# Sirui-Xu/InterDiff

Measured on AMD Instinct MI355X. Metric: denoising frame-steps/sec (denoising-steps/sec x B x T frames), higher is better.
Workload: dtype f32 (every contraction of the denoiser -- feed-forward block, QKV projection, self-attention, row-block contractions and the two token GEMMs: every fp32 operand as two f16 planes, 3 f16 MFMAs per product, fp32 accumulate; SMPL and everything else fp32 MFMA / VALU)

## Files before the change

include/interdiff_hip.h:

```cpp
#ifndef INTERDIFF_HIP_H
#define INTERDIFF_HIP_H

#include <stddef.h>
#include <stdint.h>

#ifdef __cplusplus
extern "C" {
#endif

#define IDF_OK            0
#define IDF_E_INVAL      -22
#define IDF_E_NOMEM      -12
#define IDF_E_LAUNCH     -5

int         interdiff_abi_version(void);
const char *interdiff_build_info(void);

int interdiff_rotation_6d_to_matrix   (const float *d6, float *m,  int64_t n, void *stream);
int interdiff_matrix_to_rotation_6d   (const float *m,  float *d6, int64_t n, void *stream);
int interdiff_matrix_to_axis_angle    (const float *m,  float *aa, int64_t n, void *stream);
int interdiff_axis_angle_to_matrix    (const float *aa, float *m,  int64_t n, void *stream);
int interdiff_axis_angle_to_quaternion(const float *aa, float *q,  int64_t n, void *stream);
int interdiff_rotation_6d_to_axis_angle(const float *d6, float *aa, int64_t n, void *stream);

typedef struct {
    int32_t V, J, n_betas, KB, S;
    const float   *blend;
    const float   *jt;
    const float   *js;
    const int32_t *parents;
    const int32_t *skin_idx;
    const float   *skin_w;
} idf_smpl_model;

size_t interdiff_smpl_workspace_bytes(const idf_smpl_model *m, int64_t N);
int interdiff_smpl_forward(const idf_smpl_model *m, const float *pose, const float *betas,
                           const float *trans, int64_t N, float *verts, float *jtr,
                           float *v_posed, void *ws, size_t ws_bytes, void *stream);

int interdiff_vertex_normals(const float *verts, int64_t N, int32_t V, const int32_t *faces,
                             const int32_t *adj_ptr, const int32_t *adj_face,
                             const int32_t *adj_corner, float *normals, void *stream);
int interdiff_nn_argmin(const float *q, int32_t Pq, const float *r, int32_t Pr, int64_t N,
                        int32_t *idx, void *stream);
int interdiff_point2point_signed(const float *x, int32_t P1, const float *y, int32_t P2, int64_t N,
                                 const float *x_normals, const float *y_normals,
                                 float *y2x_signed, float *x2y_signed, int32_t *yidx, int32_t *xidx,
                                 float *y2x, float *x2y, void *stream);

#define IDF_MDM_LAYERS 8
#define IDF_MDM_D      256
#define IDF_MDM_FF     1024
#define IDF_MDM_HEADS  4
#define IDF_MDM_NQ     10
#define IDF_MDM_MEM    10
#define IDF_MDM_MEM_MAX 16
#define IDF_FFN_SLICES 5

typedef struct {
    int64_t is_qan;
    int64_t sa_in_w, sa_in_b, sa_out_w, sa_out_b;
    int64_t qc, wk;
    int64_t ca_q_w, ca_q_b;
    int64_t ca_kv_w, ca_kv_b;
    int64_t ca_out_w, ca_out_b;
    int64_t ff1_w, ff1_b, ff2_w, ff2_b;
    int64_t ffn_pack;
    int64_t ffn_b1p;
    int64_t sa_in_pack;
    int64_t sa_out_frag;
    int64_t ln_w[3], ln_b[3];
    int64_t ffn_pack_h2;
    int64_t sa_in_pack_h2;
    int64_t qc_h2;
    int64_t rb_h2_ok;
    int64_t sa_out_frag_h2;
    int64_t qkv_bounds_ok;
} idf_mdm_layer;

typedef struct {
    int32_t C;
    int32_t n_steps;
    const float *arena;
    int64_t in_w, in_b;
    int64_t out_w, out_b;
    int64_t temb_table;
    int64_t pe;
    int32_t max_T, has_encoder;
    idf_mdm_layer layer[IDF_MDM_LAYERS];
    idf_mdm_layer enc_layer[IDF_MDM_LAYERS];
    int32_t tune[8];
    int64_t out_w_h2, in_w_h2;
    int64_t tail_h2_ok;
    int32_t mem_len;
    int32_t rb_tokens;
} idf_mdm_weights;

int interdiff_gemm_f32(const float *A, int32_t lda, const float *W, const float *bias, const float *resid, float *C,
                       int32_t ldc, int32_t M, int32_t N, int32_t K, int32_t epi, int32_t cfg, void *stream);

int interdiff_mdm_ffn(const idf_mdm_weights *w, int32_t layer, int32_t encoder, const float *x2, int32_t M, float *parts, void *stream);
size_t interdiff_mdm_memctx_floats_for(int32_t B, int32_t mem_len);

size_t interdiff_mdm_memctx_floats(int32_t B);
size_t interdiff_mdm_workspace_bytes(int32_t B, int32_t T);
int interdiff_mdm_prepare_memory(const idf_mdm_weights *w, const float *cond, int32_t B,
                                 float *memctx, void *ws, size_t ws_bytes, void *stream);
int interdiff_mdm_forward(const idf_mdm_weights *w, const float *memctx, const float *x,
                          const int64_t *ts, int32_t B, int32_t T, float *x0,
                          void *ws, size_t ws_bytes, void *stream);

typedef struct {
    int64_t w[3], b[3];
    int32_t c[4];
} idf_pn_mlp;

typedef struct {
    const float *arena;
    idf_pn_mlp sa1[2];
    idf_pn_mlp sa2[2];
    int64_t lin_w, lin_b;
} idf_pointnet2;

int interdiff_pointnet2_encode(const idf_pointnet2 *pn, const float *obj_points, int32_t B, int32_t P, float *out,
                               void *stream);
size_t interdiff_mdm_encode_workspace_bytes(int32_t B, int32_t Tp);
int interdiff_mdm_encode(const idf_mdm_weights *w, const float *pc, const float *x_past, int32_t B, int32_t Tp,
                         float *cond, void *ws, size_t ws_bytes, void *stream);

int interdiff_inpaint(float *x0, const float *gt, const uint8_t *mask, int64_t n, void *stream);
int interdiff_posterior_step(float *x, const float *x0, const float *noise, int64_t n,
                             float c1, float c2, float sigma, uint64_t seed, uint64_t step_index,
                             void *stream);
int interdiff_randn(float *out, int64_t n, uint64_t seed, uint64_t step_index, void *stream);
int interdiff_posterior_step_at(float *x, const float *x0, const float *noise, int64_t n,
                                float c1, float c2, float sigma, uint64_t seed, uint64_t step_index,
                                uint64_t elem0, void *stream);
int interdiff_randn_at(float *out, int64_t n, uint64_t seed, uint64_t step_index, uint64_t elem0, void *stream);
int interdiff_posterior_step_dev(float *x, const float *x0, const float *gt, const uint8_t *mask, int64_t n,
                                 const float *table, int64_t *state, int64_t *ts, int32_t B, void *stream);
int interdiff_sampler_advance(int64_t *state, int64_t *ts, int32_t B, void *stream);
int interdiff_mdm_forward_step(const idf_mdm_weights *w, const float *memctx, float *x, int64_t *ts, int32_t B, int32_t T,
                               const float *gt, const uint8_t *mask, const float *table, int64_t *state,
                               void *ws, size_t ws_bytes, void *stream);
#define IDF_STEP_EMBED_READY 1
#define IDF_STEP_EMBED_NEXT 2
int interdiff_mdm_forward_step_ex(const idf_mdm_weights *w, const float *memctx, float *x, int64_t *ts, int32_t B, int32_t T,
                                  const float *gt, const uint8_t *mask, const float *table, int64_t *state, void *ws,
                                  size_t ws_bytes, int32_t flags, void *stream);
int interdiff_mdm_step_chaining(const idf_mdm_weights *w);
int interdiff_exclusive_cu_report(char *buf, int32_t cap);
int interdiff_debug_deny_exclusive(const char *patterns);

typedef struct {
    int32_t T, past_len, P, n_pre;
    const float *arena;
    int64_t dct_pad;
    int64_t dct;
    int64_t idct;
    int64_t hand_bonus;
    int64_t layer[12];
    int32_t cin[12], cout[12];
} idf_objproj;

int interdiff_objprojector_sample(const idf_objproj *op, const float *obj_angles,
                                  const float *obj_trans, const float *markers,
                                  const int32_t *contact, int32_t B, float *out, void *stream);

typedef struct {
    const idf_smpl_model *smpl;
    const idf_objproj    *objproj;
    const int32_t *faces;
    const int32_t *adj_ptr, *adj_face, *adj_corner;
    const int32_t *markers_idx;
    int32_t n_markers, n_points, past_len;
    int32_t tune;
    const int32_t *vorder, *faces_scan, *markers_scan, *adj_pair_scan;
    const int32_t *adj_pair;
    const int32_t *vrank;
} idf_correction_ctx;

size_t interdiff_correction_workspace_bytes(const idf_correction_ctx *c, int32_t B, int32_t T);
int interdiff_correction(const idf_correction_ctx *c, float *x0, const float *gt,
                         const float *hand_pose, const float *beta, const float *obj_points,
                         int32_t B, int32_t T, float blend_t ,
                         uint8_t *condition, int32_t *contact, float *distance, float *loss,
                         void *ws, size_t ws_bytes, void *stream);
int interdiff_correction_dev(const idf_correction_ctx *c, float *x0, const float *gt, const float *hand_pose,
                             const float *beta, const float *obj_points, int32_t B, int32_t T, const float *table,
                             const int64_t *state, void *ws, size_t ws_bytes, void *stream);

#define IDF_CONTACT_STATS 12
size_t interdiff_contact_nn_workspace_bytes(const idf_correction_ctx *c, int32_t B, int32_t T);
int interdiff_contact_nn(const idf_correction_ctx *c, const float *verts, const float *obj_points, const float *objR,
                         const float *objT, int32_t B, int32_t T, float *o2h, int32_t *idx, uint64_t *stats,
                         void *ws, size_t ws_bytes, void *stream);

size_t interdiff_metrics_workspace_bytes(const idf_correction_ctx *c, int32_t B, int32_t T);
int interdiff_metrics(const idf_correction_ctx *c, const float *obj_pred, const float *jtr,
                      const float *body_trans, const float *obj_gt, const float *jtr_gt,
                      const float *body_trans_gt, const float *verts, const float *obj_points,
                      int32_t B, int32_t T, int32_t J, float *out6 ,
                      void *ws, size_t ws_bytes, void *stream);

typedef struct {
    int32_t T, past_len, J, n_pre;
    const float *arena;
    int64_t dct_pad;
    int64_t dct;
    int64_t idct;
    int64_t layer[12];
    int32_t cin[12], cout[12];
} idf_skel_objproj;

int interdiff_skeleton_objprojector_sample(const idf_skel_objproj *op, const float *obj_angles,
                                           const float *obj_trans, const float *human_points, int32_t B,
                                           float *quat_out, float *trans_out, void *stream);
int interdiff_skeleton_correction(const idf_skel_objproj *op, const float *x, const float *gt,
                                  const float *zero_pose_obj, int32_t B, int32_t T, float blend_t,
                                  float *out, void *stream);
int interdiff_skeleton_metrics(const float *body_pred, const float *body_gt, const float *obj_pred,
                               const float *obj_gt, const float *pose_pred, const float *pose_gt,
                               int32_t T, int32_t B, int32_t from_frame, float *out4, void *stream);

#define IDF_OPT_NP 483
#define IDF_OPT_NLOSS 6
typedef struct {
    const idf_correction_ctx *geo;
    const float   *blendT;
    const int32_t *jv_ptr;
    const int32_t *jv_vtx;
    const float   *jv_w;
    int32_t K3P, _pad;
} idf_opt_ctx;

typedef struct {
    int32_t B, T, P, max_iters;
    const float *betas;
    const float *obj_points;
    float *param, *init, *grad, *m, *v, *best;
    float *pose, *tr;
    float *verts, *vposed, *verts_gt, *gv;
    float *jtr;
    float *pts, *y2x;
    float *y2x_signed;
    int32_t *yidx;
    int32_t *near;
    float *dvposed;
    float *dA;
    float *dfeat;
    float *gtr;
    float *lossf;
    float *loss;
    float *loss_hist;
    float *best_loss;
    int32_t *flag;
    uint8_t *foot_static;
    int32_t *foot_cnt;
    int32_t *ctl;
    void *smpl_ws; size_t smpl_ws_bytes;
    int32_t *porder; float *psort, *pbox;
} idf_opt_state;

int interdiff_optimize_init(const idf_opt_ctx *c, const idf_opt_state *st, const float *pose, const float *trans,
                            const float *obj_angles, const float *obj_trans, int32_t first_iter, void *stream);
int interdiff_optimize_loss_grad(const idf_opt_ctx *c, const idf_opt_state *st, void *stream);
int interdiff_optimize_step(const idf_opt_ctx *c, const idf_opt_state *st, void *stream);
int interdiff_optimize_finish(const idf_opt_ctx *c, const idf_opt_state *st, float *pose, float *trans, float *obj_angles,
                              float *obj_trans, void *stream);
int interdiff_debug_joint_map_vjp(const float *R, const float *g_out, float *g_in, int32_t n);
int interdiff_debug_lds_sentinel(uint32_t *out, int32_t n_wg, int32_t spin, void *stream);
int interdiff_debug_f16_aggressor(const float *src, size_t n_floats, float *sink, int32_t iters, int32_t grid, int32_t with_loads, void *stream);

enum {
    IDF_K_EMBED = 0, IDF_K_GEMM_QKV, IDF_K_SELF_ATTN, IDF_K_GEMM_OUTPROJ, IDF_K_ROWBLOCK_QAN,
    IDF_K_ROWBLOCK_STD, IDF_K_FFN_FUSED, IDF_K_RESERVED7, IDF_K_GEMM_HEADS, IDF_K_MEM_PREP,
    IDF_K_INPAINT, IDF_K_POSTERIOR, IDF_K_CORR_PREPARE, IDF_K_SMPL_POSE, IDF_K_SMPL_BLEND_SKIN,
    IDF_K_CORR_CONTACT, IDF_K_CORR_REDUCE, IDF_K_OBJPROJ, IDF_K_CORR_BLEND, IDF_K_OTHER,
    IDF_K_COUNT
};
int interdiff_profile_begin(int32_t capacity);
int interdiff_profile_end(double *ms_per_kind, int64_t *count_per_kind);

enum {
    IDF_TUNE_FFN = 3, IDF_TUNE_FFN_MATH = 4, IDF_TUNE_COUNT = 8
};

#ifdef __cplusplus
}
#endif
#endif
```

interdiff_amd/_lib.py:

```python
import ctypes as C
import os
import torch

_HERE = os.path.dirname(os.path.abspath(__file__))
LIB_PATH = os.environ.get('INTERDIFF_HIP_LIB') or os.path.join(_HERE, 'csrc', 'libinterdiff_hip.so')
ABI_VERSION = 17

vp, i32, i64, f32, u64, sz = C.c_void_p, C.c_int32, C.c_int64, C.c_float, C.c_uint64, C.c_size_t

MDM_LAYERS = 8
FFN_SLICES = 5
STEP_EMBED_READY, STEP_EMBED_NEXT = 1, 2
TUNE = dict(ffn=3, ffn_math=4)


class SmplModel(C.Structure):
    _fields_ = [('V', i32), ('J', i32), ('n_betas', i32), ('KB', i32), ('S', i32),
                ('blend', vp), ('jt', vp), ('js', vp), ('parents', vp), ('skin_idx', vp), ('skin_w', vp)]


class MdmLayer(C.Structure):
    _fields_ = [('is_qan', i64),
                ('sa_in_w', i64), ('sa_in_b', i64), ('sa_out_w', i64), ('sa_out_b', i64),
                ('qc', i64), ('wk', i64),
                ('ca_q_w', i64), ('ca_q_b', i64), ('ca_kv_w', i64), ('ca_kv_b', i64),
                ('ca_out_w', i64), ('ca_out_b', i64),
                ('ff1_w', i64), ('ff1_b', i64), ('ff2_w', i64), ('ff2_b', i64), ('ffn_pack', i64), ('ffn_b1p', i64), ('sa_in_pack', i64), ('sa_out_frag', i64),
                ('ln_w', i64 * 3), ('ln_b', i64 * 3), ('ffn_pack_h2', i64), ('sa_in_pack_h2', i64), ('qc_h2', i64), ('rb_h2_ok', i64), ('sa_out_frag_h2', i64), ('qkv_bounds_ok', i64)]


class MdmWeights(C.Structure):
    _fields_ = [('C', i32), ('n_steps', i32), ('arena', vp),
                ('in_w', i64), ('in_b', i64), ('out_w', i64), ('out_b', i64),
                ('temb_table', i64), ('pe', i64), ('max_T', i32), ('has_encoder', i32),
                ('layer', MdmLayer * MDM_LAYERS), ('enc_layer', MdmLayer * MDM_LAYERS), ('tune', i32 * 8), ('out_w_h2', i64), ('in_w_h2', i64), ('tail_h2_ok', i64), ('mem_len', i32), ('rb_tokens', i32)]


class PnMlp(C.Structure):
    _fields_ = [('w', i64 * 3), ('b', i64 * 3), ('c', i32 * 4)]


class PointNet2(C.Structure):
    _fields_ = [('arena', vp), ('sa1', PnMlp * 2), ('sa2', PnMlp * 2), ('lin_w', i64), ('lin_b', i64)]


class ObjProj(C.Structure):
    _fields_ = [('T', i32), ('past_len', i32), ('P', i32), ('n_pre', i32), ('arena', vp),
                ('dct_pad', i64), ('dct', i64), ('idct', i64), ('hand_bonus', i64),
                ('layer', i64 * 12), ('cin', i32 * 12), ('cout', i32 * 12)]


class SkelObjProj(C.Structure):
    _fields_ = [('T', i32), ('past_len', i32), ('J', i32), ('n_pre', i32), ('arena', vp),
                ('dct_pad', i64), ('dct', i64), ('idct', i64),
                ('layer', i64 * 12), ('cin', i32 * 12), ('cout', i32 * 12)]


class CorrectionCtx(C.Structure):
    _fields_ = [('smpl', C.POINTER(SmplModel)), ('objproj', C.POINTER(ObjProj)),
                ('faces', vp), ('adj_ptr', vp), ('adj_face', vp), ('adj_corner', vp), ('markers_idx', vp),
                ('n_markers', i32), ('n_points', i32), ('past_len', i32), ('tune', i32),
                ('vorder', vp), ('faces_scan', vp), ('markers_scan', vp), ('adj_pair_scan', vp), ('adj_pair', vp), ('vrank', vp)]


class OptCtx(C.Structure):
    _fields_ = [('geo', C.POINTER(CorrectionCtx)), ('blendT', vp), ('jv_ptr', vp), ('jv_vtx', vp), ('jv_w', vp), ('K3P', i32), ('_pad', i32)]


OPT_NP, OPT_NLOSS = 483, 6
_OPT_PTRS = ('betas', 'obj_points', 'param', 'init', 'grad', 'm', 'v', 'best', 'pose', 'tr', 'verts', 'vposed', 'verts_gt', 'gv',
             'jtr', 'pts', 'y2x', 'y2x_signed', 'yidx', 'near', 'dvposed', 'dA', 'dfeat', 'gtr', 'lossf', 'loss', 'loss_hist',
             'best_loss', 'flag', 'foot_static', 'foot_cnt', 'ctl', 'smpl_ws')


class OptState(C.Structure):
    _fields_ = [('B', i32), ('T', i32), ('P', i32), ('max_iters', i32)] + [(k, vp) for k in _OPT_PTRS] + [('smpl_ws_bytes', sz), ('porder', vp), ('psort', vp), ('pbox', vp)]


_SIGS = {
    'interdiff_abi_version': (C.c_int, []),
    'interdiff_build_info': (C.c_char_p, []),
    'interdiff_rotation_6d_to_matrix': (C.c_int, [vp, vp, i64, vp]),
    'interdiff_matrix_to_rotation_6d': (C.c_int, [vp, vp, i64, vp]),
    'interdiff_matrix_to_axis_angle': (C.c_int, [vp, vp, i64, vp]),
    'interdiff_axis_angle_to_matrix': (C.c_int, [vp, vp, i64, vp]),
    'interdiff_axis_angle_to_quaternion': (C.c_int, [vp, vp, i64, vp]),
    'interdiff_rotation_6d_to_axis_angle': (C.c_int, [vp, vp, i64, vp]),
    'interdiff_smpl_workspace_bytes': (sz, [C.POINTER(SmplModel), i64]),
    'interdiff_smpl_forward': (C.c_int, [C.POINTER(SmplModel), vp, vp, vp, i64, vp, vp, vp, vp, sz, vp]),
    'interdiff_vertex_normals': (C.c_int, [vp, i64, i32, vp, vp, vp, vp, vp, vp]),
    'interdiff_nn_argmin': (C.c_int, [vp, i32, vp, i32, i64, vp, vp]),
    'interdiff_point2point_signed': (C.c_int, [vp, i32, vp, i32, i64, vp, vp, vp, vp, vp, vp, vp, vp, vp]),
    'interdiff_gemm_f32': (C.c_int, [vp, i32, vp, vp, vp, vp, i32, i32, i32, i32, i32, i32, vp]),
    'interdiff_pointnet2_encode': (C.c_int, [C.POINTER(PointNet2), vp, i32, i32, vp, vp]),
    'interdiff_mdm_encode_workspace_bytes': (sz, [i32, i32]),
    'interdiff_mdm_encode': (C.c_int, [C.POINTER(MdmWeights), vp, vp, i32, i32, vp, vp, sz, vp]),
    'interdiff_mdm_ffn': (C.c_int, [C.POINTER(MdmWeights), i32, i32, vp, i32, vp, vp]),
    'interdiff_mdm_memctx_floats': (sz, [i32]),
    'interdiff_mdm_memctx_floats_for': (sz, [i32, i32]),
    'interdiff_mdm_workspace_bytes': (sz, [i32, i32]),
    'interdiff_mdm_prepare_memory': (C.c_int, [C.POINTER(MdmWeights), vp, i32, vp, vp, sz, vp]),
    'interdiff_mdm_forward': (C.c_int, [C.POINTER(MdmWeights), vp, vp, vp, i32, i32, vp, vp, sz, vp]),
    'interdiff_mdm_forward_step': (C.c_int, [C.POINTER(MdmWeights), vp, vp, vp, i32, i32, vp, vp, vp, vp, vp, sz, vp]),
    'interdiff_mdm_forward_step_ex': (C.c_int, [C.POINTER(MdmWeights), vp, vp, vp, i32, i32, vp, vp, vp, vp, vp, sz, i32, vp]),
    'interdiff_mdm_step_chaining': (C.c_int, [C.POINTER(MdmWeights)]),
    'interdiff_inpaint': (C.c_int, [vp, vp, vp, i64, vp]),
    'interdiff_posterior_step': (C.c_int, [vp, vp, vp, i64, f32, f32, f32, u64, u64, vp]),
    'interdiff_randn': (C.c_int, [vp, i64, u64, u64, vp]),
    'interdiff_posterior_step_at': (C.c_int, [vp, vp, vp, i64, f32, f32, f32, u64, u64, u64, vp]),
    'interdiff_randn_at': (C.c_int, [vp, i64, u64, u64, u64, vp]),
    'interdiff_posterior_step_dev': (C.c_int, [vp, vp, vp, vp, i64, vp, vp, vp, i32, vp]),
    'interdiff_sampler_advance': (C.c_int, [vp, vp, i32, vp]),
    'interdiff_objprojector_sample': (C.c_int, [C.POINTER(ObjProj), vp, vp, vp, vp, i32, vp, vp]),
    'interdiff_correction_workspace_bytes': (sz, [C.POINTER(CorrectionCtx), i32, i32]),
    'interdiff_correction': (C.c_int, [C.POINTER(CorrectionCtx), vp, vp, vp, vp, vp, i32, i32, f32,
                                       vp, vp, vp, vp, vp, sz, vp]),
    'interdiff_correction_dev': (C.c_int, [C.POINTER(CorrectionCtx), vp, vp, vp, vp, vp, i32, i32, vp, vp, vp, sz, vp]),
    'interdiff_metrics_workspace_bytes': (sz, [C.POINTER(CorrectionCtx), i32, i32]),
    'interdiff_metrics': (C.c_int, [C.POINTER(CorrectionCtx), vp, vp, vp, vp, vp, vp, vp, vp, i32, i32, i32,
                                    vp, vp, sz, vp]),
    'interdiff_contact_nn_workspace_bytes': (sz, [C.POINTER(CorrectionCtx), i32, i32]),
    'interdiff_contact_nn': (C.c_int, [C.POINTER(CorrectionCtx), vp, vp, vp, vp, i32, i32, vp, vp, vp, vp, sz, vp]),
    'interdiff_skeleton_objprojector_sample': (C.c_int, [C.POINTER(SkelObjProj), vp, vp, vp, i32, vp, vp, vp]),
    'interdiff_skeleton_correction': (C.c_int, [C.POINTER(SkelObjProj), vp, vp, vp, i32, i32, f32, vp, vp]),
    'interdiff_skeleton_metrics': (C.c_int, [vp, vp, vp, vp, vp, vp, i32, i32, i32, vp, vp]),
    'interdiff_optimize_init': (C.c_int, [C.POINTER(OptCtx), C.POINTER(OptState), vp, vp, vp, vp, i32, vp]),
    'interdiff_optimize_loss_grad': (C.c_int, [C.POINTER(OptCtx), C.POINTER(OptState), vp]),
    'interdiff_optimize_step': (C.c_int, [C.POINTER(OptCtx), C.POINTER(OptState), vp]),
    'interdiff_optimize_finish': (C.c_int, [C.POINTER(OptCtx), C.POINTER(OptState), vp, vp, vp, vp, vp]),
    'interdiff_debug_joint_map_vjp': (C.c_int, [vp, vp, vp, i32]),
    'interdiff_debug_lds_sentinel': (C.c_int, [vp, i32, i32, vp]),
    'interdiff_exclusive_cu_report': (C.c_int, [C.c_char_p, i32]),
    'interdiff_debug_deny_exclusive': (C.c_int, [C.c_char_p]),
    'interdiff_debug_f16_aggressor': (C.c_int, [vp, sz, vp, i32, i32, i32, vp]),
    'interdiff_profile_begin': (C.c_int, [i32]),
    'interdiff_profile_end': (C.c_int, [C.POINTER(C.c_double), C.POINTER(C.c_int64)]),
}

KERNEL_KINDS = ('embed', 'gemm_qkv', 'self_attn', 'gemm_outproj', 'rowblock_qan', 'rowblock_std', 'ffn_fused', 'reserved7',
                'gemm_heads', 'mem_prep', 'inpaint', 'posterior', 'corr_prepare', 'smpl_pose', 'smpl_blend_skin',
                'corr_contact', 'corr_reduce', 'objproj', 'corr_blend', 'other')

_lib = None


class HipLibraryMissing(RuntimeError):
    pass


def load():
    global _lib
    if _lib is not None:
        return _lib
    if not os.path.exists(LIB_PATH):
        raise HipLibraryMissing('%s not found: build it with `python -m interdiff_amd.csrc.build` '
                                '(there is no CPU/torch fallback for the hot path)' % LIB_PATH)
    lib = C.CDLL(LIB_PATH)
    for name, (res, args) in _SIGS.items():
        fn = getattr(lib, name)
        fn.restype, fn.argtypes = res, args
    if lib.interdiff_abi_version() != ABI_VERSION:
        raise HipLibraryMissing('stale %s: abi %d != %d, rebuild' % (LIB_PATH, lib.interdiff_abi_version(), ABI_VERSION))
    _lib = lib
    return lib


def exclusive_cu_report():
    buf = C.create_string_buffer(8192)
    bad = load().interdiff_exclusive_cu_report(buf, len(buf))
    if bad < 0:
        check(bad, 'exclusive_cu_report')
    return buf.value.decode(), bad


def debug_deny_exclusive(patterns=''):
    check(load().interdiff_debug_deny_exclusive(patterns.encode() if patterns else None), 'debug_deny_exclusive')


def exported_symbols():
    return sorted(_SIGS)


_ERR = {-22: 'IDF_E_INVAL (bad shape / pointer / unsupported size)', -12: 'IDF_E_NOMEM (workspace too small)',
        -5: 'IDF_E_LAUNCH (kernel launch failed)'}


def check(rc, what=''):
    if rc != 0:
        raise RuntimeError('interdiff_hip %s failed: %s' % (what, _ERR.get(rc, rc)))


def dptr(t, dtype=None, allow_none=False):
    if t is None:
        if allow_none:
            return vp(None)
        raise ValueError('null tensor')
    if not t.is_cuda:
        raise ValueError('interdiff_amd ops need device tensors (got %s); the HIP path has no CPU fallback' % t.device)
    if not t.is_contiguous():
        raise ValueError('tensor must be contiguous')
    if dtype is not None and t.dtype != dtype:
        raise ValueError('expected %s, got %s' % (dtype, t.dtype))
    return vp(t.data_ptr())


def stream():
    return vp(torch.cuda.current_stream().cuda_stream)
```

interdiff_amd/correction.py:

```python
import ctypes as C
import os
import itertools
import numpy as np
import torch
from . import _lib
from .geometry import MeshTopology

MARKERS67 = [3470, 3171, 3327, 857, 1812, 628, 182, 3116, 3040, 239,
             1666, 1725, 0, 2174, 1568, 1368, 3387, 2112, 1053, 1058,
             3336, 3346, 1323, 2108, 3122, 3314, 1252, 1082, 1861, 1454,
             850, 2224, 3233, 1769, 6728, 4343, 5273, 4116, 3694, 6399,
             6540, 6488, 3749, 5135, 5194, 3512, 5635, 5210, 4360, 4841,
             6786, 5573, 4538, 4544, 6736, 6747, 4804, 5568, 6544, 6682,
             5322, 4927, 5686, 4598, 6633, 3506, 3508]


_UID = itertools.count(1)


def correction_gate(t0):
    return not (t0 > 500 or t0 % 50 != 0)


class HipCorrection:
    def __init__(self, smpl_layer, objprojector, n_points=2048, past_len=10, markers=MARKERS67, device='cuda', scan_order=True):
        self.lib = _lib.load()
        self.device = torch.device(device)
        self.smpl, self.objproj, self.past_len = smpl_layer, objprojector, past_len
        self.topo = MeshTopology(smpl_layer.th_faces, smpl_layer.cmodel.V, self.device, rest_vertices=getattr(smpl_layer, 'v_template', None) if scan_order else None)
        self.markers_idx = torch.tensor(list(markers), dtype=torch.int32, device=self.device)
        ctx = _lib.CorrectionCtx()
        ctx.smpl = C.pointer(smpl_layer.cmodel)
        ctx.objproj = C.pointer(objprojector.cop)
        ctx.faces, ctx.adj_ptr = self.topo.faces.data_ptr(), self.topo.adj_ptr.data_ptr()
        ctx.adj_face, ctx.adj_corner = self.topo.adj_face.data_ptr(), self.topo.adj_corner.data_ptr()
        ctx.markers_idx = self.markers_idx.data_ptr()
        ctx.n_markers, ctx.n_points, ctx.past_len = len(markers), n_points, past_len
        if self.topo.vorder is not None:
            self.markers_scan = self.topo.scan_positions(markers, self.device)
            ctx.vorder, ctx.faces_scan, ctx.markers_scan = self.topo.vorder.data_ptr(), self.topo.faces_scan.data_ptr(), self.markers_scan.data_ptr()
            ctx.adj_pair_scan = self.topo.adj_pair_scan.data_ptr()
            ctx.vrank = self.topo.vrank.data_ptr()
        ctx.tune = 0
        self.ctx = ctx
        self._ws = {}
        self.debug = None
        self._uid = next(_UID)

    graph_capturable = True

    def workspace_for(self, B, T):
        return torch.empty(self.lib.interdiff_correction_workspace_bytes(C.byref(self.ctx), B, T), dtype=torch.uint8, device=self.device)

    def apply_dev(self, x, table, state, y, ws):
        B, _, Cc, T = x.shape
        if y['obj_points'].shape[1] != self.ctx.n_points:
            raise ValueError('obj_points must have %d points' % self.ctx.n_points)
        _lib.check(self.lib.interdiff_correction_dev(C.byref(self.ctx), _lib.dptr(x, torch.float32), _lib.dptr(y['inpainted_motion'], torch.float32),
                                                     _lib.dptr(y['hand_pose'], torch.float32), _lib.dptr(y['beta'], torch.float32),
                                                     _lib.dptr(y['obj_points'], torch.float32), B, T, _lib.dptr(table), _lib.dptr(state),
                                                     _lib.dptr(ws), ws.numel(), _lib.stream()), 'correction_dev')
        return x

    def _workspace(self, B, T):
        need = self.lib.interdiff_correction_workspace_bytes(C.byref(self.ctx), B, T)
        key = torch.cuda.current_stream(self.device).cuda_stream
        ws = self._ws.pop(key, None)
        if ws is None or ws.numel() < need:
            ws = torch.empty(need, dtype=torch.uint8, device=self.device)
        self._ws[key] = ws
        if len(self._ws) > self.MAX_STREAM_WORKSPACES:
            torch.cuda.synchronize(self.device)
            self._ws.pop(next(iter(self._ws)))
        return ws

    MAX_STREAM_WORKSPACES = 4

    @staticmethod
    def slice_kwargs(model_kwargs, sl):
        y = model_kwargs['y']
        per_clip_dim = dict(inpainted_motion=0, inpainting_mask=0, obj_points=0, hand_pose=1, beta=1, cond=1)
        ys = {k: (v[(slice(None),) * per_clip_dim[k] + (sl,)].contiguous() if k in per_clip_dim and isinstance(v, torch.Tensor) else v) for k, v in y.items()}
        return dict(model_kwargs, y=ys)

    def apply(self, x, t0, y):
        B, _, Cc, T = x.shape
        if not x.is_contiguous():
            raise ValueError('x must be contiguous (it is updated in place)')
        if y['obj_points'].shape[1] != self.ctx.n_points:
            raise ValueError('obj_points must have %d points' % self.ctx.n_points)
        gt = y['inpainted_motion'].contiguous()
        hp, beta, pts = y['hand_pose'].contiguous().float(), y['beta'].contiguous().float(), y['obj_points'].contiguous().float()
        ws = self._workspace(B, T)
        dbg = [None] * 4
        if self.debug is not None:
            dbg = [torch.empty(B, dtype=torch.uint8, device=self.device), torch.empty(B, len(MARKERS67), dtype=torch.int32, device=self.device),
                   torch.empty(B, device=self.device), torch.empty(B, device=self.device)]
        blend_t = float(np.float32(t0) / np.float32(1000))
        _lib.check(self.lib.interdiff_correction(C.byref(self.ctx), _lib.dptr(x, torch.float32), _lib.dptr(gt, torch.float32),
                                                 _lib.dptr(hp), _lib.dptr(beta), _lib.dptr(pts), B, T, blend_t,
                                                 *[_lib.dptr(d, allow_none=True) for d in dbg], _lib.dptr(ws), ws.numel(),
                                                 _lib.stream()), 'correction')
        if self.debug is not None:
            self.debug.update(condition=dbg[0], contact=dbg[1], distance=dbg[2], loss=dbg[3])
        return x

    def contact_nn(self, verts, obj_points, objR, objT, want_stats=False):
        T, B = verts.shape[:2]
        P = self.ctx.n_points
        o2h = torch.empty(T, B, P, device=self.device)
        idx = torch.empty(T, B, P, dtype=torch.int32, device=self.device)
        stats = torch.zeros(12, dtype=torch.int64, device=self.device) if want_stats else None
        need = self.lib.interdiff_contact_nn_workspace_bytes(C.byref(self.ctx), B, T)
        ws = getattr(self, '_nn_ws', None)
        if ws is None or ws.numel() < need:
            ws = self._nn_ws = torch.empty(need, dtype=torch.uint8, device=self.device)
        v, pts, R_, t_ = (a.contiguous().float() for a in (verts, obj_points, objR, objT))
        _lib.check(self.lib.interdiff_contact_nn(C.byref(self.ctx), _lib.dptr(v), _lib.dptr(pts), _lib.dptr(R_), _lib.dptr(t_), B, T, _lib.dptr(o2h),
                                                 _lib.dptr(idx), _lib.dptr(stats, allow_none=True), _lib.dptr(ws), ws.numel(), _lib.stream()), 'contact_nn')
        return (o2h, idx, tuple(int(x) for x in stats.cpu())) if want_stats else (o2h, idx)

    def is_active(self, t0):
        return correction_gate(int(t0))

    def __call__(self, x, t, model_kwargs):
        t0 = getattr(t, 'host_value', None)
        if t0 is None:
            t0 = int(t[0])
        if not correction_gate(t0):
            return x
        return self.apply(x, t0, model_kwargs['y'])
```

interdiff_amd/csrc/correction.hip:

```cpp
#include "common.h"
#include "objproj.h"
#include "rot_math.h"
#include <float.h>

namespace {

constexpr int NBODY = 22;
constexpr int CTOK = 144;

__global__ __launch_bounds__(256) void corr_prepare_kernel(const float *__restrict__ x0, const float *__restrict__ gt,
                                                           const float *__restrict__ hand_pose, int B, int T,
                                                           float *__restrict__ pose, float *__restrict__ trans,
                                                           float *__restrict__ objR, float *__restrict__ objT,
                                                           float *__restrict__ gt_angles, float *__restrict__ gt_trans) {
    const int64_t i = (int64_t)blockIdx.x * 256 + threadIdx.x;
    const int64_t N = (int64_t)B * T;
    if (i >= N * 24) return;
    const int64_t n = i / 24;
    const int slot = (int)(i - n * 24), t = (int)(n / B), b = (int)(n - (int64_t)t * B);
    const float *xb = x0 + (size_t)b * CTOK * T + t;
    if (slot < NBODY) {
        float d[6], m[9], a[3];
#pragma unroll
        for (int k = 0; k < 6; ++k) d[k] = xb[(size_t)(slot * 6 + k) * T];
        rot::rot6d_to_matrix(d, m);
        rot::matrix_to_axis_angle(m, a);
        float *p = pose + n * 156 + slot * 3;
        p[0] = a[0]; p[1] = a[1]; p[2] = a[2];
    } else if (slot == 22) {
        for (int k = 0; k < 90; ++k) pose[n * 156 + 66 + k] = hand_pose[n * 90 + k];
#pragma unroll
        for (int k = 0; k < 3; ++k) trans[n * 3 + k] = xb[(size_t)(132 + k) * T];
    } else {
        float d[6], m[9];
#pragma unroll
        for (int k = 0; k < 6; ++k) d[k] = xb[(size_t)(135 + k) * T];
        rot::rot6d_to_matrix(d, m);
#pragma unroll
        for (int k = 0; k < 9; ++k) objR[n * 9 + k] = m[k];
        const float *gb = gt + (size_t)b * CTOK * T + t;
#pragma unroll
        for (int k = 0; k < 3; ++k) {
            objT[n * 3 + k] = xb[(size_t)(141 + k) * T];
            gt_trans[n * 3 + k] = gb[(size_t)(141 + k) * T];
        }
#pragma unroll
        for (int k = 0; k < 6; ++k) gt_angles[n * 6 + k] = gb[(size_t)(135 + k) * T];
    }
}

__device__ __forceinline__ float dist2_exact(float qx, float qy, float qz, float rx, float ry, float rz) {
#pragma clang fp contract(off)
    const float dx = qx - rx, dy = qy - ry, dz = qz - rz;
    const float xx = dx * dx, yy = dy * dy, zz = dz * dz;
    return (xx + yy) + zz;
}

__device__ __forceinline__ float3 f3(const float4 v) { return make_float3(v.x, v.y, v.z); }
__device__ __forceinline__ float3 sub3(float3 a, float3 b) { return make_float3(a.x - b.x, a.y - b.y, a.z - b.z); }
__device__ __forceinline__ float3 cross3(float3 a, float3 b) {
    return make_float3(a.y * b.z - a.z * b.y, a.z * b.x - a.x * b.z, a.x * b.y - a.y * b.x);
}

constexpr int MAXP = 2048;
__global__ __launch_bounds__(1024) void corr_point_order_kernel(const float *__restrict__ obj_points, int P, int32_t *__restrict__ porder) {
    __shared__ unsigned long long keys[MAXP];
    __shared__ float red[6][1024];
    const int b = blockIdx.x, tid = threadIdx.x;
    const float *op = obj_points + (size_t)b * P * 3;
    float p[2][3];
    float lo[3] = {FLT_MAX, FLT_MAX, FLT_MAX}, hi[3] = {-FLT_MAX, -FLT_MAX, -FLT_MAX};
#pragma unroll
    for (int k = 0; k < 2; ++k) {
        const int i = tid + 1024 * k;
#pragma unroll
        for (int a = 0; a < 3; ++a) {
            p[k][a] = i < P ? op[3 * i + a] : 0.f;
            if (i < P) { lo[a] = fminf(lo[a], p[k][a]); hi[a] = fmaxf(hi[a], p[k][a]); }
        }
    }
#pragma unroll
    for (int a = 0; a < 3; ++a) { red[a][tid] = lo[a]; red[3 + a][tid] = hi[a]; }
    __syncthreads();
    for (int s = 512; s > 0; s >>= 1) {
        if (tid < s) {
#pragma unroll
            for (int a = 0; a < 3; ++a) {
                red[a][tid] = fminf(red[a][tid], red[a][tid + s]);
                red[3 + a][tid] = fmaxf(red[3 + a][tid], red[3 + a][tid + s]);
            }
        }
        __syncthreads();
    }
#pragma unroll
    for (int k = 0; k < 2; ++k) {
        const int i = tid + 1024 * k;
        unsigned long long key = ~0ull;
        if (i < P) {
            unsigned code = 0;
            unsigned q[3];
#pragma unroll
            for (int a = 0; a < 3; ++a) {
                const float ext = red[3 + a][0] - red[a][0];
                const float u = ext > 0.f ? (p[k][a] - red[a][0]) / ext : 0.f;
                q[a] = (unsigned)fminf(fmaxf(u * 1023.0f, 0.f), 1023.0f);
            }
#pragma unroll
            for (int bit = 0; bit < 10; ++bit)
#pragma unroll
                for (int a = 0; a < 3; ++a) code |= ((q[a] >> bit) & 1u) << (3 * bit + a);
            key = ((unsigned long long)code << 11) | (unsigned)i;
        }
        keys[i] = key;
    }
    __syncthreads();
    for (int k = 2; k <= MAXP; k <<= 1) {
        for (int j = k >> 1; j > 0; j >>= 1) {
            const int l = 2 * j * (tid / j) + (tid % j), r = l + j;
            const unsigned long long x = keys[l], y = keys[r];
            const bool up = (l & k) == 0;
            if ((x > y) == up) { keys[l] = y; keys[r] = x; }
            __syncthreads();
        }
    }
#pragma unroll
    for (int k = 0; k < 2; ++k) {
        const int i = tid + 1024 * k;
        if (i < P) porder[(size_t)b * P + i] = (int32_t)(keys[i] & 2047u);
    }
}

constexpr int MAXM = 128;
constexpr float MARK_D2 = 0.00039999996079131961f;
constexpr int CB = 16;
constexpr int SB = 8;
constexpr int SEED_STRIDE = 4;
constexpr int CT = 1024;
constexpr int TASK = 64;
typedef float v2f __attribute__((ext_vector_type(2)));

struct ContactLds {
    int V4, nCB, nSB, nSeed;
    int rec, mark, box, sbox, seed, flags, red, pl, total;
    __host__ __device__ explicit ContactLds(int V) {
        V4 = (V + CB - 1) / CB * CB; nCB = V4 / CB; nSB = (nCB + SB - 1) / SB; nSeed = (nCB + SEED_STRIDE - 1) / SEED_STRIDE;
        rec = 0;
        mark = rec + V4;
        box = mark + MAXM;
        sbox = box + 3 * (nSB * SB / 2);
        seed = sbox + 3 * ((nSB + 2) / 2);
        flags = seed + 2 * ((nSeed + 1) / 2);
        red = flags + MAXM / 4;
        pl = red + CT / 4;
        total = pl + MAXP / 4;
    }
};

__device__ __forceinline__ float3 lds_rec(const float4 *vs, int pos) {
    const float *f = reinterpret_cast<const float *>(vs + 2 * (pos >> 1));
    const int h = pos & 1;
    return make_float3(f[h], f[2 + h], f[4 + h]);
}
__device__ __forceinline__ void lds_rec_store(float4 *vs, int pos, float x, float y, float z) {
    float *f = reinterpret_cast<float *>(vs + 2 * (pos >> 1));
    const int h = pos & 1;
    f[h] = x; f[2 + h] = y; f[4 + h] = z;
}
__device__ __forceinline__ void lds_box_store(float4 *bx, int k, float3 lo, float3 hi) {
    float *f = reinterpret_cast<float *>(bx + 3 * (k >> 1));
    const int h = k & 1;
    f[h] = lo.x; f[2 + h] = lo.y; f[4 + h] = lo.z; f[6 + h] = hi.x; f[8 + h] = hi.y; f[10 + h] = hi.z;
}
__device__ __forceinline__ void lds_box_load(const float4 *bx, int k, float3 &lo, float3 &hi) {
    const float *f = reinterpret_cast<const float *>(bx + 3 * (k >> 1));
    const int h = k & 1;
    lo = make_float3(f[h], f[2 + h], f[4 + h]);
    hi = make_float3(f[6 + h], f[8 + h], f[10 + h]);
}

struct PredArgs {
    idf_objproj op;
    const float *obj_angles, *obj_trans;
    const int32_t *markers_idx;
    float *markers, *keep;
    int nclips;
};
template <bool OPT, bool WITH_PRED = false>
__global__ __launch_bounds__(CT) void corr_contact_kernel(const float *__restrict__ verts, int V,
                                                          const float *__restrict__ obj_points, int P,
                                                          const int32_t *__restrict__ porder ,
                                                          const float *__restrict__ objR, const float *__restrict__ objT,
                                                          const int32_t *__restrict__ faces ,
                                                          const int32_t *__restrict__ adj_ptr,
                                                          const int32_t *__restrict__ adj_face,
                                                          const int32_t *__restrict__ adj_corner,
                                                          const int32_t *__restrict__ adj_pair ,
                                                          const int32_t *__restrict__ vorder ,
                                                          const int32_t *__restrict__ vrank ,
                                                          const int32_t *__restrict__ markers_pos , int M, int B,
                                                          float *__restrict__ markers_out, float *__restrict__ loss_sum,
                                                          float *__restrict__ min_dist, int32_t *__restrict__ label,
                                                          float *__restrict__ o2h_out ,
                                                          int32_t *__restrict__ idx_out ,
                                                          unsigned long long *__restrict__ stats ,
                                                          int64_t nn_from ,
                                                          const float *__restrict__ pts_frame , int frames_per_clip ,
                                                          const PredArgs pred) {
    extern __shared__ __attribute__((aligned(16))) float4 vs[];
    if constexpr (WITH_PRED) {
        if ((int)blockIdx.x < pred.nclips) {
            const int b = blockIdx.x, Tn = pred.op.T;
            for (int i = threadIdx.x; i < Tn * M; i += CT) {
                const int t = i / M, m = i - t * M;
                const size_t nfr = (size_t)t * B + b;
                const float *v = verts + (nfr * V + pred.markers_idx[m]) * 3;
                float *o = pred.markers + (nfr * M + m) * 3;
                o[0] = v[0]; o[1] = v[1]; o[2] = v[2];
            }
            __threadfence();
            __syncthreads();
            idf_objproj_dev::objproj_body<1>(reinterpret_cast<float *>(vs), pred.op, pred.obj_angles, pred.obj_trans, pred.markers, nullptr, B, b, pred.keep, nullptr);
            return;
        }
    }
    const ContactLds L(V);
    const int nCB = L.nCB, nSB = L.nSB;
    float4 *ms = vs + L.mark, *bb = vs + L.box, *sbb = vs + L.sbox, *sd = vs + L.seed;
    int *flags = reinterpret_cast<int *>(vs + L.flags);
    float *red = reinterpret_cast<float *>(vs + L.red);
    float *pl = reinterpret_cast<float *>(vs + L.pl);
    __shared__ int next_task;
    const int64_t n = WITH_PRED ? (int64_t)blockIdx.x - pred.nclips : (int64_t)blockIdx.x;
    const int b = OPT ? (int)(n / frames_per_clip) : (int)(n % B), tid = threadIdx.x;
    const float *vf = verts + (size_t)n * V * 3;
    const bool do_nn = n >= nn_from;
    long long t_prev = 0;
    int n_phase = 0;
    auto phase_done = [&]() {
        if (stats && tid == 0 && do_nn) {
            const long long now = (long long)__builtin_readcyclecounter();
            if (n_phase > 0) atomicAdd(stats + 3 + n_phase, (unsigned long long)(now - t_prev));
            t_prev = now;
        }
        ++n_phase;
    };
    phase_done();
    float R[9] = {1.f, 0.f, 0.f, 0.f, 1.f, 0.f, 0.f, 0.f, 1.f}, tr[3] = {0.f, 0.f, 0.f};
    if constexpr (!OPT) {
#pragma unroll
        for (int k = 0; k < 9; ++k) R[k] = objR[n * 9 + k];
#pragma unroll
        for (int k = 0; k < 3; ++k) tr[k] = objT[n * 3 + k];
    }
    const int my_marker_pos = (!OPT && tid < M) ? markers_pos[tid] : 0;
    if (vorder && vrank) {
        for (int i0 = tid; i0 < V; i0 += 4 * CT) {
            typedef float f3v __attribute__((ext_vector_type(3), aligned(4)));
            int pos[4];
            f3v pv[4];
#pragma unroll
            for (int k = 0; k < 4; ++k) {
                const int i = min(i0 + k * CT, V - 1);
                pos[k] = vrank[i];
                pv[k] = *reinterpret_cast<const f3v *>(vf + 3 * i);
            }
#pragma unroll
            for (int k = 0; k < 4; ++k) {
                if (i0 + k * CT < V) {
                    lds_rec_store(vs, pos[k], pv[k].x, pv[k].y, pv[k].z);
                    reinterpret_cast<int *>(vs + 2 * (pos[k] >> 1) + 1)[2 + (pos[k] & 1)] = i0 + k * CT;
                }
            }
        }
        for (int v = V + tid; v < L.V4; v += CT) {
            lds_rec_store(vs, v, 3e18f, 3e18f, 3e18f);
            reinterpret_cast<int *>(vs + 2 * (v >> 1) + 1)[2 + (v & 1)] = 0x7fffffff;
        }
    } else
    for (int v0 = tid; v0 < L.V4; v0 += 4 * CT) {
        int o[4];
        float x[4], y[4], z[4];
#pragma unroll
        for (int k = 0; k < 4; ++k) {
            const int v = v0 + k * CT;
            o[k] = v < V ? (vorder ? vorder[v] : v) : -1;
        }
#pragma unroll
        for (int k = 0; k < 4; ++k) {
            x[k] = y[k] = z[k] = 3e18f;
            if (o[k] >= 0) {
                typedef float f3v __attribute__((ext_vector_type(3), aligned(4)));
                const f3v pv = *reinterpret_cast<const f3v *>(vf + 3 * o[k]);
                x[k] = pv.x; y[k] = pv.y; z[k] = pv.z;
            }
        }
#pragma unroll
        for (int k = 0; k < 4; ++k) {
            const int v = v0 + k * CT;
            if (v < L.V4) {
                lds_rec_store(vs, v, x[k], y[k], z[k]);
                reinterpret_cast<int *>(vs + 2 * (v >> 1) + 1)[2 + (v & 1)] = o[k] >= 0 ? o[k] : 0x7fffffff;
            }
        }
    }
    if (tid < MAXM) flags[tid] = 0;
    const int ntask_all = (P + TASK - 1) / TASK;
    const int task0 = (int)((long long)blockIdx.y * ntask_all / gridDim.y), task1 = (int)((long long)(blockIdx.y + 1) * ntask_all / gridDim.y);
    if (tid == 0) next_task = task0;
    for (int i = tid; i < MAXP; i += CT) pl[i] = 0.f;
    __syncthreads();
    phase_done();
    if (!OPT && tid < ((M + 1) & ~1)) {
        float3 mk = make_float3(3e18f, 3e18f, 3e18f);
        if (tid < M) {
            mk = lds_rec(vs, my_marker_pos);
            if (markers_out) {
                float *mo = markers_out + ((size_t)n * M + tid) * 3;
                mo[0] = mk.x; mo[1] = mk.y; mo[2] = mk.z;
            }
        }
        lds_rec_store(ms, tid, mk.x, mk.y, mk.z);
    }
    if (do_nn) {
#define IDF_DPP8(v, op, ctrl) v = op(v, __builtin_bit_cast(float, __builtin_amdgcn_update_dpp(__builtin_bit_cast(int, v), __builtin_bit_cast(int, v), ctrl, 0xf, 0xf, false)))
        const int lane_ = tid & 63, wave_ = tid >> 6, nsw = 2 * ((nSB + 2) / 2);
        for (int sb = wave_; sb < nsw; sb += CT / 64) {
            const int pr = sb * 64 + lane_;
            float lx = FLT_MAX, ly = FLT_MAX, lz = FLT_MAX, hx = -FLT_MAX, hy = -FLT_MAX, hz = -FLT_MAX;
            if (2 * pr < V) {
                const float4 xy = vs[2 * pr], zz = vs[2 * pr + 1];
                const bool two = 2 * pr + 1 < V;
                lx = two ? fminf(xy.x, xy.y) : xy.x; hx = two ? fmaxf(xy.x, xy.y) : xy.x;
                ly = two ? fminf(xy.z, xy.w) : xy.z; hy = two ? fmaxf(xy.z, xy.w) : xy.z;
                lz = two ? fminf(zz.x, zz.y) : zz.x; hz = two ? fmaxf(zz.x, zz.y) : zz.x;
            }
            IDF_DPP8(lx, fminf, 0xB1); IDF_DPP8(lx, fminf, 0x4E); IDF_DPP8(lx, fminf, 0x141);
            IDF_DPP8(ly, fminf, 0xB1); IDF_DPP8(ly, fminf, 0x4E); IDF_DPP8(ly, fminf, 0x141);
            IDF_DPP8(lz, fminf, 0xB1); IDF_DPP8(lz, fminf, 0x4E); IDF_DPP8(lz, fminf, 0x141);
            IDF_DPP8(hx, fmaxf, 0xB1); IDF_DPP8(hx, fmaxf, 0x4E); IDF_DPP8(hx, fmaxf, 0x141);
            IDF_DPP8(hy, fmaxf, 0xB1); IDF_DPP8(hy, fmaxf, 0x4E); IDF_DPP8(hy, fmaxf, 0x141);
            IDF_DPP8(hz, fmaxf, 0xB1); IDF_DPP8(hz, fmaxf, 0x4E); IDF_DPP8(hz, fmaxf, 0x141);
            const int cb = sb * SB + (lane_ >> 3);
            if ((lane_ & 7) == 0 && cb < nSB * SB) lds_box_store(bb, cb, make_float3(lx, ly, lz), make_float3(hx, hy, hz));
            const float slx = -wave_max(-lx), sly = -wave_max(-ly), slz = -wave_max(-lz), shx = wave_max(hx), shy = wave_max(hy), shz = wave_max(hz);
            if (lane_ == 0) lds_box_store(sbb, sb, make_float3(slx, sly, slz), make_float3(shx, shy, shz));
        }
#undef IDF_DPP8
        for (int k = tid; k < 2 * ((L.nSeed + 1) / 2); k += CT) {
            const float3 p = lds_rec(vs, min(k * SEED_STRIDE, nCB - 1) * CB);
            lds_rec_store(sd, k, p.x, p.y, p.z);
        }
    }
    const float *op = OPT ? pts_frame + (size_t)n * P * 3 : obj_points + (size_t)b * P * 3;
    const int ln = tid & 63, ntask = task1;
    __syncthreads();
    phase_done();
    float mind2 = FLT_MAX;
    unsigned n_exec = 0, n_test = 0, n_tasks = 0;
    for (;;) {
        int task = 0;
        if (ln == 0) task = atomicAdd(&next_task, 1);
        task = __builtin_amdgcn_readfirstlane(task);
        if (task >= ntask) break;
        ++n_tasks;
        const int sp = task * TASK + ln;
        const int i = sp < P ? (porder ? porder[(size_t)b * P + sp] : sp) : -1;
        const bool valid = i >= 0;
        float px = 0.f, py = 0.f, pz = 0.f;
        if (valid) { px = op[3 * i]; py = op[3 * i + 1]; pz = op[3 * i + 2]; }
        const float qx = OPT ? px : (px * R[0] + py * R[1] + pz * R[2]) + tr[0];
        const float qy = OPT ? py : (px * R[3] + py * R[4] + pz * R[5]) + tr[1];
        const float qz = OPT ? pz : (px * R[6] + py * R[7] + pz * R[8]) + tr[2];
        if (do_nn) {
#pragma clang fp contract(off)
            const v2f QX = v2f{qx, qx}, QY = v2f{qy, qy}, QZ = v2f{qz, qz};
            auto pair_d2 = [&](const float4 xy, const float4 zz) {
#pragma clang fp contract(off)
                const v2f dx = QX - v2f{xy.x, xy.y}, dy = QY - v2f{xy.z, xy.w}, dz = QZ - v2f{zz.x, zz.y};
                return (dx * dx + dy * dy) + dz * dz;
            };
            auto pair_a2 = [&](const float4 xy, const float2 zz) {
                const v2f dx = QX - v2f{xy.x, xy.y}, dy = QY - v2f{xy.z, xy.w}, dz = QZ - v2f{zz.x, zz.y};
                return __builtin_elementwise_fma(dz, dz, __builtin_elementwise_fma(dy, dy, dx * dx));
            };
            constexpr float SCAN_M = 1.000003814697265625f, SCAN_ABS = 1e-37f;
            float seed = FLT_MAX;
            for (int k = 0; k < (L.nSeed + 1) / 2; k += 4) {
                float4 xy[4]; float2 zz[4];
#pragma unroll
                for (int u = 0; u < 4; ++u) { xy[u] = sd[2 * min(k + u, (L.nSeed + 1) / 2 - 1)]; zz[u] = *reinterpret_cast<const float2 *>(&sd[2 * min(k + u, (L.nSeed + 1) / 2 - 1) + 1]); }
#pragma unroll
                for (int u = 0; u < 4; ++u) {
                    const v2f a2 = pair_a2(xy[u], zz[u]);
                    seed = fminf(fminf(seed, a2.x), a2.y);
                }
            }
            float thr = __builtin_fmaf(seed, SCAN_M, SCAN_ABS);
            float best = FLT_MAX, bthr = FLT_MAX;
            int tie = 0;
            int bblk = 0, bblk2 = 0;
            auto pair_lb = [&](const float4 a, const float4 bq, const float4 c) {
#pragma clang fp contract(off)
                const v2f ax = v2f{a.x, a.y} - QX, bx = QX - v2f{bq.z, bq.w};
                const v2f ay = v2f{a.z, a.w} - QY, by = QY - v2f{c.x, c.y};
                const v2f az = v2f{bq.x, bq.y} - QZ, bz = QZ - v2f{c.z, c.w};
                const v2f ex = v2f{fmaxf(fmaxf(ax.x, bx.x), 0.f), fmaxf(fmaxf(ax.y, bx.y), 0.f)};
                const v2f ey = v2f{fmaxf(fmaxf(ay.x, by.x), 0.f), fmaxf(fmaxf(ay.y, by.y), 0.f)};
                const v2f ez = v2f{fmaxf(fmaxf(az.x, bz.x), 0.f), fmaxf(fmaxf(az.y, bz.y), 0.f)};
                return __builtin_elementwise_fma(ez, ez, __builtin_elementwise_fma(ey, ey, ex * ex));
            };
            auto score_block = [&](int cb) {
                ++n_exec;
                const int v0 = cb * CB;
                float4 xy[CB / 2]; float2 zz[CB / 2];
#pragma unroll
                for (int u = 0; u < CB / 2; ++u) { xy[u] = vs[v0 + 2 * u]; zz[u] = *reinterpret_cast<const float2 *>(&vs[v0 + 2 * u + 1]); }
                float bm = FLT_MAX;
#pragma unroll
                for (int u = 0; u < CB / 2; ++u) {
                    const v2f a2 = pair_a2(xy[u], zz[u]);
                    bm = fminf(fminf(bm, a2.x), a2.y);
                }
                if (bm < best) {
                    const float w = __builtin_fmaf(bm, SCAN_M, SCAN_ABS);
                    if (best <= w) { tie = tie ? 2 : 1; bblk2 = bblk; } else tie = 0;
                    best = bm; bblk = v0; bthr = w; thr = fminf(thr, w);
                } else if (bm <= bthr) { tie = tie ? 2 : 1; bblk2 = v0; }
            };
            auto scan_super = [&](int sb) {
                const int cb0 = sb * SB;
#pragma unroll
                for (int j = 0; j < SB / 2; ++j) {
                    const int cb = cb0 + 2 * j;
                    const float4 *bx = bb + 3 * (cb >> 1);
                    const v2f lb = pair_lb(bx[0], bx[1], bx[2]);
                    n_test += 2;
                    if (__builtin_amdgcn_ballot_w64(valid && lb.x <= thr) != 0ull) score_block(cb);
                    if (__builtin_amdgcn_ballot_w64(valid && lb.y <= thr) != 0ull) score_block(cb + 1);
                }
            };
            if (!vorder) {
                for (int cb = 0; cb < nCB; ++cb) score_block(cb);
            } else
            for (int sb = 0; sb < nSB; sb += 2) {
                const float4 *bx = sbb + 3 * (sb >> 1);
                const v2f lb = pair_lb(bx[0], bx[1], bx[2]);
                n_test += 2;
                if (__builtin_amdgcn_ballot_w64(valid && lb.x <= thr) != 0ull) scan_super(sb);
                if (__builtin_amdgcn_ballot_w64(valid && lb.y <= thr) != 0ull) scan_super(sb + 1);
            }
            int pos = bblk, org = 0x7fffffff;
            float ebest = FLT_MAX;
            auto resolve_pair = [&](int pr) {
                const float4 xy = vs[2 * pr], zz = vs[2 * pr + 1];
                const v2f d2 = pair_d2(xy, zz);
                const int o0 = __builtin_bit_cast(int, zz.z), o1 = __builtin_bit_cast(int, zz.w);
                if (d2.x < ebest || (d2.x == ebest && o0 < org)) { ebest = d2.x; org = o0; pos = 2 * pr; }
                if (d2.y < ebest || (d2.y == ebest && o1 < org)) { ebest = d2.y; org = o1; pos = 2 * pr + 1; }
            };
            if (tie < 2) {
#pragma unroll
                for (int u = 0; u < CB / 2; ++u) resolve_pair((bblk >> 1) + u);
                if (tie) {
#pragma unroll
                    for (int u = 0; u < CB / 2; ++u) resolve_pair((bblk2 >> 1) + u);
                }
            } else {
                for (int pr = 0; pr < (V + 1) / 2; ++pr) resolve_pair(pr);
            }
            pos = min(pos, V - 1);
            if (org == 0x7fffffff) org = vorder ? vorder[pos] : pos;
            if constexpr (OPT) {
                if (valid) idx_out[(size_t)n * P + i] = org;
            } else if (valid) {
                const float3 v3 = lds_rec(vs, pos);
                float3 acc = make_float3(0.f, 0.f, 0.f);
                const int e0 = adj_ptr[org], e1 = adj_ptr[org + 1];
                if (adj_pair) {
                    for (int e = e0; e < e1; e += 4) {
                        int2 ab[4];
#pragma unroll
                        for (int u = 0; u < 4; ++u) ab[u] = *reinterpret_cast<const int2 *>(adj_pair + 2 * (size_t)min(e + u, e1 - 1));
#pragma unroll
                        for (int u = 0; u < 4; ++u) {
                            if (e + u < e1) {
                                const float3 nn = cross3(sub3(lds_rec(vs, ab[u].x), v3), sub3(lds_rec(vs, ab[u].y), v3));
                                acc.x += nn.x; acc.y += nn.y; acc.z += nn.z;
                            }
                        }
                    }
                } else {
                    for (int e = e0; e < e1; ++e) {
                        const int f = adj_face[e], c = adj_corner[e];
                        const float3 p0 = lds_rec(vs, faces[3 * f]), p1 = lds_rec(vs, faces[3 * f + 1]), p2 = lds_rec(vs, faces[3 * f + 2]);
                        float3 nn;
                        if (c == 1) nn = cross3(sub3(p2, p1), sub3(p0, p1));
                        else if (c == 2) nn = cross3(sub3(p0, p2), sub3(p1, p2));
                        else nn = cross3(sub3(p1, p0), sub3(p2, p0));
                        acc.x += nn.x; acc.y += nn.y; acc.z += nn.z;
                    }
                }
                const float nl = fmaxf(sqrtf(acc.x * acc.x + acc.y * acc.y + acc.z * acc.z), 1e-6f);
                const float vx = qx - v3.x, vy = qy - v3.y, vz = qz - v3.z;
                const float dt = (acc.x / nl) * vx + (acc.y / nl) * vy + (acc.z / nl) * vz;
                const float d = sqrtf(vx * vx + vy * vy + vz * vz);
                const float o2h = d * (dt > 0.f ? 1.f : (dt < 0.f ? -1.f : 0.f));
                if (o2h_out) o2h_out[(size_t)n * P + i] = o2h;
                if (idx_out) idx_out[(size_t)n * P + i] = org;
                pl[sp] = o2h < 0.f ? fabsf(o2h) * 20.0f : 0.f;
            }
        }
        if (!OPT && valid) {
#pragma clang fp contract(off)
            const v2f QX = v2f{qx, qx}, QY = v2f{qy, qy}, QZ = v2f{qz, qz};
            for (int p2 = 0; p2 < (M + 1) / 2; ++p2) {
                const float4 xy = ms[2 * p2], zz = ms[2 * p2 + 1];
                const v2f dx = v2f{xy.x, xy.y} - QX, dy = v2f{xy.z, xy.w} - QY, dz = v2f{zz.x, zz.y} - QZ;
                const v2f d2 = __builtin_elementwise_fma(dy, dy, dx * dx) + dz * dz;
                mind2 = fminf(fminf(mind2, d2.x), d2.y);
                if (__builtin_amdgcn_ballot_w64(fminf(d2.x, d2.y) < MARK_D2) != 0ull) {
                    if (d2.x < MARK_D2) flags[2 * p2] = 1;
                    if (d2.y < MARK_D2) flags[2 * p2 + 1] = 1;
                }
            }
        }
    }
    if (stats && ln == 0 && do_nn) {
        atomicAdd(stats, (unsigned long long)n_exec);
        atomicAdd(stats + 1, (unsigned long long)nCB * n_tasks);
        atomicAdd(stats + 2, (unsigned long long)n_test);
    }
    phase_done();
    if constexpr (OPT) return;
    __syncthreads();
    phase_done();
    float loss = 0.f;
#pragma unroll
    for (int k = 0; k < MAXP / CT; ++k) loss += pl[tid + CT * k];
    red[tid] = loss;
    __syncthreads();
    for (int s = CT / 2; s > 0; s >>= 1) {
        if (tid < s) red[tid] += red[tid + s];
        __syncthreads();
    }
    const float loss_total = red[0];
    __syncthreads();
    red[tid] = mind2;
    __syncthreads();
    for (int s = CT / 2; s > 0; s >>= 1) {
        if (tid < s) red[tid] = fminf(red[tid], red[tid + s]);
        __syncthreads();
    }
    if (tid == 0) { loss_sum[n] = loss_total; min_dist[n] = red[0] == FLT_MAX ? FLT_MAX : sqrtf(red[0]); }
    if (tid < M) label[(size_t)n * M + tid] = flags[tid];
    phase_done();
    if (stats && tid == 0 && do_nn) atomicAdd(stats + 3, 1ull);
}

size_t contact_lds_bytes(int V) { return (size_t)ContactLds(V).total * sizeof(float4); }

int launch_contact(hipStream_t s, int64_t N, const float *verts, int V, const float *obj_points, int P, int32_t *porder,
                   const float *objR, const float *objT, const idf_correction_ctx *c, int B, float *markers, float *loss_sum,
                   float *min_dist, int32_t *label, float *o2h, int32_t *idx, unsigned long long *stats, int64_t nn_from, const PredArgs *pred = nullptr) {
    const int M = c->n_markers;
    const size_t lds = contact_lds_bytes(V);
    if (lds > 160 * 1024 - 16384 || P > MAXP) return IDF_E_INVAL;
    const bool ordered = c->vorder != nullptr;
    if (ordered != (c->faces_scan != nullptr) || ordered != (c->markers_scan != nullptr) || ordered != (c->adj_pair_scan != nullptr)) return IDF_E_INVAL;
    const int32_t *faces = ordered ? c->faces_scan : c->faces, *mpos = ordered ? c->markers_scan : c->markers_idx;
    if (porder) hipLaunchKernelGGL(corr_point_order_kernel, dim3((unsigned)B), dim3(1024), 0, s, obj_points, P, porder);
    if (pred) {
        const size_t lds2 = (pred->nclips > 0 && lds < idf_objproj_dev::OBJPROJ_LDS) ? idf_objproj_dev::OBJPROJ_LDS : lds;
        static std::atomic<uint64_t> lds_ok2{0};
        if (lds2 > 160 * 1024 - 2048) return IDF_E_INVAL;
        if (idf_opt_in_lds(reinterpret_cast<const void *>(corr_contact_kernel<false, true>), 160 * 1024 - 2048, lds_ok2) != IDF_OK) return IDF_E_LAUNCH;
        hipLaunchKernelGGL((corr_contact_kernel<false, true>), dim3((unsigned)(N + pred->nclips)), dim3(CT), lds2, s, verts, V, obj_points, P, porder, objR, objT, faces,
                           c->adj_ptr, c->adj_face, c->adj_corner, c->adj_pair_scan, c->vorder, c->vrank, mpos, M, B, markers, loss_sum, min_dist, label, o2h, idx,
                           stats, nn_from, nullptr, 0, *pred);
        return IDF_OK;
    }
    static std::atomic<uint64_t> lds_ok{0};
    if (idf_opt_in_lds(reinterpret_cast<const void *>(corr_contact_kernel<false>), 160 * 1024 - 16384, lds_ok) != IDF_OK) return IDF_E_LAUNCH;
    hipLaunchKernelGGL(corr_contact_kernel<false>, dim3((unsigned)N), dim3(CT), lds, s, verts, V, obj_points, P, porder, objR, objT, faces,
                       c->adj_ptr, c->adj_face, c->adj_corner, c->adj_pair_scan, c->vorder, c->vrank, mpos, M, B, markers, loss_sum, min_dist, label, o2h, idx,
                       stats, nn_from, nullptr, 0, PredArgs{});
    return IDF_OK;
}

__global__ __launch_bounds__(128) void corr_reduce_kernel(const float *__restrict__ loss_sum, const float *__restrict__ min_dist,
                                                          const int32_t *__restrict__ label, int B, int T, int past, int P, int M,
                                                          uint8_t *__restrict__ condition, int32_t *__restrict__ contact,
                                                          float *__restrict__ distance_out, float *__restrict__ loss_out) {
    extern __shared__ float fr[];
    const int b = blockIdx.x, tid = threadIdx.x;
    for (int t = tid; t < T; t += 128) {
        fr[t] = loss_sum[(size_t)t * B + b];
        fr[T + t] = min_dist[(size_t)t * B + b];
    }
    if (tid < M) {
        int c = 0;
#pragma unroll 16
        for (int t = past; t < T; ++t) c += label[((size_t)t * B + b) * M + tid];
        contact[(size_t)b * M + tid] = c;
    }
    __syncthreads();
    if (tid == 0) {
        float ls = 0.f, ds = 0.f;
        for (int t = past; t < T; ++t) ls += fr[t] / (float)P;
        for (int t = 0; t < T; ++t) ds += fr[T + t];
        const float loss = ls / (float)(T - past), dist = ds / (float)T;
        condition[b] = !((loss < 0.002f) && (dist < 0.02f));
        if (distance_out) distance_out[b] = dist;
        if (loss_out) loss_out[b] = loss;
    }
}

__global__ __launch_bounds__(256) void corr_blend_kernel(float *__restrict__ x0, const float *__restrict__ proj,
                                                         const uint8_t *__restrict__ condition, int B, int T, float a,
                                                         const float *__restrict__ a_table, const int64_t *__restrict__ a_state) {
    if (a_table) a = a_table[a_state[0] * 4 + 3];
    const int64_t i = (int64_t)blockIdx.x * 256 + threadIdx.x;
    if (i >= (int64_t)B * CTOK * T) return;
    const int b = (int)(i / (CTOK * T)), r = (int)(i - (int64_t)b * CTOK * T), c = r / T, t = r - c * T;
    if (!condition[b]) return;
    const float x = x0[i];
    const float other = c < 135 ? x : proj[((size_t)t * B + b) * 9 + (c - 135)];
    x0[i] = a * x + (1.0f - a) * other;
}

struct CorrWs {
    float *pose, *trans, *objR, *objT, *gt_angles, *gt_trans, *verts, *jtr, *markers, *loss_sum, *min_dist, *proj, *proj_keep;
    int32_t *label, *contact, *porder;
    uint8_t *condition;
    void *smpl_ws;
    size_t smpl_ws_bytes, total;
};

CorrWs carve(const idf_correction_ctx *c, int B, int T, void *ws) {
    const int64_t N = (int64_t)B * T;
    const int V = c->smpl->V, J = c->smpl->J, M = c->n_markers;
    char *p = reinterpret_cast<char *>(ws);
    size_t off = 0;
    auto take = [&](size_t bytes) { char *r = p ? p + off : nullptr; off += idf_align(bytes); return r; };
    CorrWs w;
    w.pose = (float *)take(N * 156 * 4);
    w.trans = (float *)take(N * 3 * 4);
    w.objR = (float *)take(N * 9 * 4);
    w.objT = (float *)take(N * 3 * 4);
    w.gt_angles = (float *)take(N * 6 * 4);
    w.gt_trans = (float *)take(N * 3 * 4);
    w.verts = (float *)take((size_t)N * V * 3 * 4);
    w.jtr = (float *)take((size_t)N * J * 3 * 4);
    w.markers = (float *)take((size_t)N * M * 3 * 4);
    w.loss_sum = (float *)take(N * 4);
    w.min_dist = (float *)take(N * 4);
    w.proj = (float *)take(N * 9 * 4);
    w.label = (int32_t *)take((size_t)N * M * 4);
    w.contact = (int32_t *)take((size_t)B * M * 4);
    w.condition = (uint8_t *)take(B);
    w.porder = (int32_t *)take((size_t)B * c->n_points * 4);
    w.proj_keep = (float *)take((size_t)B * idf_objproj_keep_floats() * 4);
    w.smpl_ws_bytes = interdiff_smpl_workspace_bytes(c->smpl, N);
    w.smpl_ws = take(w.smpl_ws_bytes);
    w.total = off;
    return w;
}


constexpr int NPATCH = MAXP / 64;
__global__ __launch_bounds__(256) void opt_patch_kernel(const float *__restrict__ pts, int P, const int32_t *__restrict__ porder, int frames_per_clip,
                                                        float4 *__restrict__ psort , float4 *__restrict__ pbox ) {
    const int64_t n = blockIdx.x;
    const int b = (int)(n / frames_per_clip), tid = threadIdx.x, lane = tid & 63, wave = tid >> 6;
    const float *pn = pts + (size_t)n * P * 3;
    for (int k = wave; k < NPATCH; k += 4) {
        const int sp = 64 * k + lane;
        float x = 3e18f, y = 3e18f, z = 3e18f;
        float lx = FLT_MAX, ly = FLT_MAX, lz = FLT_MAX, hx = -FLT_MAX, hy = -FLT_MAX, hz = -FLT_MAX;
        if (sp < P) {
            const int i = porder[(size_t)b * P + sp];
            x = pn[3 * i]; y = pn[3 * i + 1]; z = pn[3 * i + 2];
            lx = hx = x; ly = hy = y; lz = hz = z;
        }
        psort[(size_t)n * MAXP + sp] = make_float4(x, y, z, 0.f);
        lx = -wave_max(-lx); ly = -wave_max(-ly); lz = -wave_max(-lz);
        hx = wave_max(hx); hy = wave_max(hy); hz = wave_max(hz);
        if (lane == 0) {
            pbox[((size_t)n * NPATCH + k) * 2] = make_float4(lx, ly, lz, 0.f);
            pbox[((size_t)n * NPATCH + k) * 2 + 1] = make_float4(hx, hy, hz, 0.f);
        }
    }
}

__global__ __launch_bounds__(256) void opt_near_kernel(const float *__restrict__ verts, int V, int P, const float4 *__restrict__ psort,
                                                       const float4 *__restrict__ pbox, const int32_t *__restrict__ vorder,
                                                       int32_t *__restrict__ near) {
    __shared__ float4 ps[MAXP];
    __shared__ float4 bx[NPATCH * 2];
    const int64_t n = blockIdx.y;
    const int tid = threadIdx.x, pos = blockIdx.x * 256 + tid, vid = vorder[min(pos, V - 1)];
    for (int i = tid; i < MAXP; i += 256) ps[i] = psort[(size_t)n * MAXP + i];
    if (tid < NPATCH * 2) bx[tid] = pbox[(size_t)n * NPATCH * 2 + tid];
    const bool valid = pos < V;
    const float *vp = verts + ((size_t)n * V + vid) * 3;
    const float vx = vp[0], vy = vp[1], vz = vp[2];
    __syncthreads();
    const int npatch = (P + 63) / 64;
    bool hit = false;
    {
#pragma clang fp contract(off)
        const v2f VX = v2f{vx, vx}, VY = v2f{vy, vy}, VZ = v2f{vz, vz};
        for (int k = 0; k < npatch; ++k) {
            if (__builtin_amdgcn_ballot_w64(valid && !hit) == 0ull) break;
            const float4 lo = bx[2 * k], hi = bx[2 * k + 1];
            const float ex = fmaxf(fmaxf(lo.x - vx, vx - hi.x), 0.f), ey = fmaxf(fmaxf(lo.y - vy, vy - hi.y), 0.f), ez = fmaxf(fmaxf(lo.z - vz, vz - hi.z), 0.f);
            const float xx = ex * ex, yy = ey * ey, zz = ez * ez;
            if (__builtin_amdgcn_ballot_w64(valid && !hit && (xx + yy) + zz < 0.25f) == 0ull) continue;
            const float4 *pp = ps + 64 * k;
            for (int j0 = 0; j0 < 64; j0 += 16) {
#pragma unroll
                for (int j = j0; j < j0 + 16; j += 2) {
                    const float4 p = pp[j], q = pp[j + 1];
                    const v2f dx = v2f{p.x, q.x} - VX, dy = v2f{p.y, q.y} - VY, dz = v2f{p.z, q.z} - VZ;
                    const v2f d2 = (dx * dx + dy * dy) + dz * dz;
                    hit = hit || d2.x < 0.25f || d2.y < 0.25f;
                }
                if (__builtin_amdgcn_ballot_w64(valid && !hit) == 0ull) break;
            }
        }
    }
    if (valid) near[(size_t)n * V + vid] = hit ? 1 : 0;
}

}

int idf_point_order(hipStream_t s, const float *obj_points, int B, int P, int32_t *porder) {
    if (P > MAXP) return IDF_E_INVAL;
    hipLaunchKernelGGL(corr_point_order_kernel, dim3((unsigned)B), dim3(1024), 0, s, obj_points, P, porder);
    return IDF_OK;
}

int idf_nn_scan_opt(hipStream_t s, int64_t N, int frames_per_clip, const float *verts, int V, const float *pts_frame, const float *obj_points, int P,
                    const int32_t *porder, const idf_correction_ctx *c, int32_t *yidx) {
    const size_t lds = contact_lds_bytes(V);
    if (lds > 160 * 1024 - 16384 || P > MAXP || !c->vorder) return IDF_E_INVAL;
    const int B = (int)(N / frames_per_clip);
    static std::atomic<uint64_t> lds_ok{0};
    if (idf_opt_in_lds(reinterpret_cast<const void *>(corr_contact_kernel<true>), 160 * 1024 - 16384, lds_ok) != IDF_OK) return IDF_E_LAUNCH;
    hipLaunchKernelGGL(corr_contact_kernel<true>, dim3((unsigned)N, 2), dim3(CT), lds, s, verts, V, obj_points, P, porder, nullptr, nullptr, nullptr,
                       nullptr, nullptr, nullptr, nullptr, c->vorder, c->vrank, nullptr, 0, B, nullptr, nullptr, nullptr, nullptr, nullptr, yidx, nullptr, (int64_t)0,
                       pts_frame, frames_per_clip, PredArgs{});
    return IDF_OK;
}

int idf_near_mask_opt(hipStream_t s, int64_t N, int frames_per_clip, const float *verts, int V, const float *pts_frame, int P, const int32_t *porder,
                      const int32_t *vorder, float *psort, float *pbox, int32_t *near) {
    if (P > MAXP || !vorder) return IDF_E_INVAL;
    hipLaunchKernelGGL(opt_patch_kernel, dim3((unsigned)N), dim3(256), 0, s, pts_frame, P, porder, frames_per_clip, reinterpret_cast<float4 *>(psort),
                       reinterpret_cast<float4 *>(pbox));
    hipLaunchKernelGGL(opt_near_kernel, dim3((unsigned)idf_cdiv(V, 256), (unsigned)N), dim3(256), 0, s, verts, V, P, reinterpret_cast<const float4 *>(psort),
                       reinterpret_cast<const float4 *>(pbox), vorder, near);
    return IDF_OK;
}

namespace {

}

extern "C" size_t interdiff_correction_workspace_bytes(const idf_correction_ctx *c, int32_t B, int32_t T) {
    if (!c || !c->smpl || B <= 0 || T <= 0) return 0;
    return carve(c, B, T, nullptr).total;
}

static int correction_impl(const idf_correction_ctx *c, float *x0, const float *gt, const float *hand_pose,
                           const float *beta, const float *obj_points, int32_t B, int32_t T, float blend_t, const float *blend_table,
                           const int64_t *blend_state, uint8_t *condition, int32_t *contact, float *distance, float *loss, void *ws,
                           size_t ws_bytes, void *stream) {
    if (!c || !c->smpl || !c->objproj || !x0 || !gt || !hand_pose || !beta || !obj_points || !ws || B <= 0 || T <= 0) return IDF_E_INVAL;
    const int V = c->smpl->V, M = c->n_markers, P = c->n_points;
    if (c->smpl->J != 52 || c->smpl->n_betas != 10 || M > MAXM || M != c->objproj->P || P > MAXP || T != c->objproj->T ||
        c->past_len != c->objproj->past_len || c->past_len >= T)
        return IDF_E_INVAL;
    CorrWs w = carve(c, B, T, ws);
    if (ws_bytes < w.total) return IDF_E_NOMEM;
    hipStream_t s = idf_stream(stream);
    const int64_t N = (int64_t)B * T;
    const bool fused = (c->tune & 2) == 0 && idf_objproj_check(c->objproj) == IDF_OK;
    idf_prof_mark(IDF_K_CORR_PREPARE, s);
    hipLaunchKernelGGL(corr_prepare_kernel, dim3((unsigned)idf_cdiv(N * 24, 256)), dim3(256), 0, s, x0, gt, hand_pose, B, T, w.pose,
                       w.trans, w.objR, w.objT, w.gt_angles, w.gt_trans);
    int rc = interdiff_smpl_forward(c->smpl, w.pose, beta, w.trans, N, w.verts, w.jtr, nullptr, w.smpl_ws, w.smpl_ws_bytes, stream);
    if (rc) return rc;
    idf_prof_mark(IDF_K_CORR_CONTACT, s);
    PredArgs pred{};
    if (fused) {
        pred.op = *c->objproj;
        pred.obj_angles = w.gt_angles; pred.obj_trans = w.gt_trans;
        pred.markers_idx = c->markers_idx; pred.markers = w.markers; pred.keep = w.proj_keep;
        pred.nclips = B;
    }
    rc = launch_contact(s, N, w.verts, V, obj_points, P, w.porder, w.objR, w.objT, c, B, fused ? nullptr : w.markers, w.loss_sum, w.min_dist, w.label, nullptr,
                        nullptr, nullptr, (int64_t)c->past_len * B, &pred);
    if (rc) return rc;
    uint8_t *cond = condition ? condition : w.condition;
    int32_t *cont = contact ? contact : w.contact;
    idf_prof_mark(IDF_K_CORR_REDUCE, s);
    hipLaunchKernelGGL(corr_reduce_kernel, dim3(B), dim3(128), 2 * (size_t)T * sizeof(float), s, w.loss_sum, w.min_dist, w.label, B, T, c->past_len, P, M, cond,
                       cont, distance, loss);
    if (fused) {
        idf_prof_mark(IDF_K_OBJPROJ, s);
        rc = idf_objproj_pick(c->objproj, w.proj_keep, cont, B, w.proj, s);
    } else {
        rc = interdiff_objprojector_sample(c->objproj, w.gt_angles, w.gt_trans, w.markers, cont, B, w.proj, stream);
    }
    if (rc) return rc;
    idf_prof_mark(IDF_K_CORR_BLEND, s);
    hipLaunchKernelGGL(corr_blend_kernel, dim3((unsigned)idf_cdiv((int64_t)B * CTOK * T, 256)), dim3(256), 0, s, x0, w.proj, cond, B, T,
                       blend_t, blend_table, blend_state);
    idf_prof_mark(-1, s);
    IDF_CHECK_LAUNCH();
    return IDF_OK;
}

extern "C" int interdiff_correction(const idf_correction_ctx *c, float *x0, const float *gt, const float *hand_pose,
                                    const float *beta, const float *obj_points, int32_t B, int32_t T, float blend_t,
                                    uint8_t *condition, int32_t *contact, float *distance, float *loss, void *ws,
                                    size_t ws_bytes, void *stream) {
    return correction_impl(c, x0, gt, hand_pose, beta, obj_points, B, T, blend_t, nullptr, nullptr, condition, contact, distance, loss, ws, ws_bytes, stream);
}

extern "C" int interdiff_correction_dev(const idf_correction_ctx *c, float *x0, const float *gt, const float *hand_pose,
                                        const float *beta, const float *obj_points, int32_t B, int32_t T, const float *table,
                                        const int64_t *state, void *ws, size_t ws_bytes, void *stream) {
    if (!table || !state) return IDF_E_INVAL;
    return correction_impl(c, x0, gt, hand_pose, beta, obj_points, B, T, 0.f, table, state, nullptr, nullptr, nullptr, nullptr, ws, ws_bytes, stream);
}

namespace {

__global__ __launch_bounds__(256) void metrics_prepare_kernel(const float *__restrict__ obj_pred, int64_t N,
                                                              float *__restrict__ objR, float *__restrict__ objT) {
    const int64_t n = (int64_t)blockIdx.x * 256 + threadIdx.x;
    if (n >= N) return;
    float q[4], m[9];
    rot::axis_angle_to_quaternion(obj_pred + n * 6, q);
    rot::quaternion_to_matrix(q, m);
#pragma unroll
    for (int k = 0; k < 9; ++k) objR[n * 9 + k] = m[k];
#pragma unroll
    for (int k = 0; k < 3; ++k) objT[n * 3 + k] = obj_pred[n * 6 + 3 + k];
}

__device__ __forceinline__ float block_sum(float v, float *red) {
    red[threadIdx.x] = v;
    __syncthreads();
    for (int s = 128; s > 0; s >>= 1) {
        if (threadIdx.x < s) red[threadIdx.x] += red[threadIdx.x + s];
        __syncthreads();
    }
    const float r = red[0];
    __syncthreads();
    return r;
}

__global__ __launch_bounds__(256) void metrics_reduce_kernel(const float *__restrict__ obj_pred, const float *__restrict__ jtr,
                                                             const float *__restrict__ body_trans, const float *__restrict__ obj_gt,
                                                             const float *__restrict__ jtr_gt, const float *__restrict__ body_trans_gt,
                                                             const float *__restrict__ o2h, int B, int T, int J, int P,
                                                             float *__restrict__ out6) {
    __shared__ float red[256];
    const int b = blockIdx.x, tid = threadIdx.x;
    float g = 0.f, l = 0.f;
    for (int i = tid; i < T * J; i += 256) {
        const int t = i / J, j = i - t * J;
        const float *a = jtr + (((size_t)t * B + b) * J + j) * 3, *c = jtr_gt + (((size_t)t * B + b) * J + j) * 3;
        const float *a0 = jtr + ((size_t)t * B + b) * J * 3, *c0 = jtr_gt + ((size_t)t * B + b) * J * 3;
        const float dx = a[0] - c[0], dy = a[1] - c[1], dz = a[2] - c[2];
        g += sqrtf(dx * dx + dy * dy + dz * dz);
        const float ex = (a[0] - a0[0]) - (c[0] - c0[0]), ey = (a[1] - a0[1]) - (c[1] - c0[1]), ez = (a[2] - a0[2]) - (c[2] - c0[2]);
        l += sqrtf(ex * ex + ey * ey + ez * ez);
    }
    float bt = 0.f, ot = 0.f, rq = 0.f;
    for (int t = tid; t < T; t += 256) {
        const size_t n = (size_t)t * B + b;
        const float *x = body_trans + n * 3, *y = body_trans_gt + n * 3;
        bt += sqrtf((x[0] - y[0]) * (x[0] - y[0]) + (x[1] - y[1]) * (x[1] - y[1]) + (x[2] - y[2]) * (x[2] - y[2]));
        const float *p = obj_pred + n * 6, *q = obj_gt + n * 6;
        ot += sqrtf((p[3] - q[3]) * (p[3] - q[3]) + (p[4] - q[4]) * (p[4] - q[4]) + (p[5] - q[5]) * (p[5] - q[5]));
        float qa[4], qb[4];
        rot::axis_angle_to_quaternion(p, qa);
        rot::axis_angle_to_quaternion(q, qb);
        float e1 = 0.f, e2 = 0.f;
#pragma unroll
        for (int k = 0; k < 4; ++k) { e1 += fabsf(qa[k] - qb[k]); e2 += fabsf(qa[k] + qb[k]); }
        rq += fminf(e1, e2);
    }
    const float gs = block_sum(g, red), ls = block_sum(l, red), bs = block_sum(bt, red), os = block_sum(ot, red), rs = block_sum(rq, red);
    float pen = 0.f;
    for (int t = 0; t < T; ++t) {
        const float *row = o2h + ((size_t)t * B + b) * P;
        float c = 0.f;
        for (int i = tid; i < P; i += 256) c += row[i] < 0.f ? 1.f : 0.f;
        const float cs = block_sum(c, red);
        pen += cs / (float)P;
    }
    if (tid == 0) {
        out6[0 * B + b] = gs / (float)J / (float)T;
        out6[1 * B + b] = ls / (float)J / (float)T;
        out6[2 * B + b] = bs / (float)T;
        out6[3 * B + b] = os / (float)T;
        out6[4 * B + b] = rs / (float)T;
        out6[5 * B + b] = pen / (float)T;
    }
}

struct MetWs {
    float *objR, *objT, *o2h, *markers, *loss_sum, *min_dist;
    int32_t *label, *porder;
    size_t total;
};
MetWs carve_metrics(const idf_correction_ctx *c, int B, int T, void *ws) {
    const int64_t N = (int64_t)B * T;
    char *p = reinterpret_cast<char *>(ws);
    size_t off = 0;
    auto take = [&](size_t bytes) { char *r = p ? p + off : nullptr; off += idf_align(bytes); return r; };
    MetWs w;
    w.objR = (float *)take(N * 9 * 4);
    w.objT = (float *)take(N * 3 * 4);
    w.o2h = (float *)take((size_t)N * c->n_points * 4);
    w.markers = (float *)take((size_t)N * c->n_markers * 3 * 4);
    w.loss_sum = (float *)take(N * 4);
    w.min_dist = (float *)take(N * 4);
    w.label = (int32_t *)take((size_t)N * c->n_markers * 4);
    w.porder = (int32_t *)take((size_t)B * c->n_points * 4);
    w.total = off;
    return w;
}

}

extern "C" size_t interdiff_contact_nn_workspace_bytes(const idf_correction_ctx *c, int32_t B, int32_t T) {
    if (!c || B <= 0 || T <= 0) return 0;
    return carve_metrics(c, B, T, nullptr).total;
}

extern "C" int interdiff_contact_nn(const idf_correction_ctx *c, const float *verts, const float *obj_points, const float *objR,
                                    const float *objT, int32_t B, int32_t T, float *o2h, int32_t *idx, uint64_t *stats, void *ws,
                                    size_t ws_bytes, void *stream) {
    if (!c || !c->smpl || !verts || !obj_points || !objR || !objT || !ws || B <= 0 || T <= 0 || (!o2h && !idx)) return IDF_E_INVAL;
    if (c->n_markers > MAXM || c->n_points > MAXP) return IDF_E_INVAL;
    MetWs w = carve_metrics(c, B, T, ws);
    if (ws_bytes < w.total) return IDF_E_NOMEM;
    hipStream_t s = idf_stream(stream);
    if (stats && hipMemsetAsync(stats, 0, IDF_CONTACT_STATS * sizeof(uint64_t), s) != hipSuccess) return IDF_E_LAUNCH;
    const int rc = launch_contact(s, (int64_t)B * T, verts, c->smpl->V, obj_points, c->n_points, w.porder, objR, objT, c, B, w.markers, w.loss_sum,
                                  w.min_dist, w.label, o2h ? o2h : w.o2h, idx, reinterpret_cast<unsigned long long *>(stats), 0);
    if (rc) return rc;
    IDF_CHECK_LAUNCH();
    return IDF_OK;
}

extern "C" size_t interdiff_metrics_workspace_bytes(const idf_correction_ctx *c, int32_t B, int32_t T) {
    if (!c || B <= 0 || T <= 0) return 0;
    return carve_metrics(c, B, T, nullptr).total;
}

extern "C" int interdiff_metrics(const idf_correction_ctx *c, const float *obj_pred, const float *jtr, const float *body_trans,
                                 const float *obj_gt, const float *jtr_gt, const float *body_trans_gt, const float *verts,
                                 const float *obj_points, int32_t B, int32_t T, int32_t J, float *out6, void *ws, size_t ws_bytes,
                                 void *stream) {
    if (!c || !c->smpl || !obj_pred || !jtr || !body_trans || !obj_gt || !jtr_gt || !body_trans_gt || !verts || !obj_points || !out6 ||
        !ws || B <= 0 || T <= 0 || J <= 0)
        return IDF_E_INVAL;
    const int V = c->smpl->V, M = c->n_markers, P = c->n_points;
    if (M > MAXM || P > MAXP) return IDF_E_INVAL;
    MetWs w = carve_metrics(c, B, T, ws);
    if (ws_bytes < w.total) return IDF_E_NOMEM;
    hipStream_t s = idf_stream(stream);
    const int64_t N = (int64_t)B * T;
    idf_prof_mark(IDF_K_OTHER, s);
    hipLaunchKernelGGL(metrics_prepare_kernel, dim3((unsigned)idf_cdiv(N, 256)), dim3(256), 0, s, obj_pred, N, w.objR, w.objT);
    const int rc = launch_contact(s, N, verts, V, obj_points, P, w.porder, w.objR, w.objT, c, B, w.markers, w.loss_sum, w.min_dist, w.label, w.o2h,
                                  nullptr, nullptr, 0);
    if (rc) return rc;
    hipLaunchKernelGGL(metrics_reduce_kernel, dim3(B), dim3(256), 0, s, obj_pred, jtr, body_trans, obj_gt, jtr_gt, body_trans_gt, w.o2h, B,
                       T, J, P, out6);
    idf_prof_mark(-1, s);
    IDF_CHECK_LAUNCH();
    return IDF_OK;
}
```

interdiff_amd/csrc/smpl.hip:

```cpp
#include "common.h"
#include "rot_math.h"
#include <algorithm>

#ifndef IDF_SMPL_STAMP
#define IDF_SMPL_STAMP(i) do { } while (0)
#endif

namespace {

constexpr int MAXJ = 64;

__global__ __launch_bounds__(64) void smpl_pose_kernel(const idf_smpl_model m, const float *__restrict__ pose,
                                                       const float *__restrict__ betas, const float *__restrict__ trans,
                                                       float *__restrict__ feat, float *__restrict__ A,
                                                       float *__restrict__ jtr) {
    __shared__ float Rs[MAXJ * 9], Js[MAXJ * 3], Gs[MAXJ * 12];
    const int64_t n = blockIdx.x;
    const int j = threadIdx.x, J = m.J, nb = m.n_betas, KB = m.KB;
    const float *beta = betas + n * nb;
    if (j < J) {
        rot::rodrigues_smpl(pose + n * 3 * J + 3 * j, Rs + j * 9);
#pragma unroll
        for (int c = 0; c < 3; ++c) {
            float s = m.jt[j * 3 + c];
            const float *jsr = m.js + (size_t)(j * 3 + c) * nb;
            for (int k = 0; k < nb; ++k) s += jsr[k] * beta[k];
            Js[j * 3 + c] = s;
        }
    }
    float *f = feat + n * KB;
    if (j >= 1 && j < J) {
#pragma unroll
        for (int e = 0; e < 9; ++e) f[(j - 1) * 9 + e] = Rs[j * 9 + e] - ((e == 0 || e == 4 || e == 8) ? 1.0f : 0.0f);
    }
    const int base = 9 * (J - 1);
    for (int k = j; k < KB - base; k += 64) f[base + k] = k < nb ? beta[k] : (k == nb ? 1.0f : 0.0f);
    __syncthreads();
    if (j < 12) {
        const int r = j >> 2, c = j & 3;
        Gs[j] = c < 3 ? Rs[r * 3 + c] : Js[r];
    }
    __syncthreads();
    for (int i = 1; i < J; ++i) {
        const int p = m.parents[i];
        if (j < 12) {
            const int r = j >> 2, c = j & 3;
            const float *gp = Gs + p * 12 + r * 4;
            float v;
            if (c < 3)
                v = gp[0] * Rs[i * 9 + c] + gp[1] * Rs[i * 9 + 3 + c] + gp[2] * Rs[i * 9 + 6 + c];
            else
                v = gp[0] * (Js[i * 3] - Js[p * 3]) + gp[1] * (Js[i * 3 + 1] - Js[p * 3 + 1]) +
                    gp[2] * (Js[i * 3 + 2] - Js[p * 3 + 2]) + gp[3];
            Gs[i * 12 + j] = v;
        }
        __syncthreads();
    }
    if (j < J) {
        const float *g = Gs + j * 12;
        const float jx = Js[j * 3], jy = Js[j * 3 + 1], jz = Js[j * 3 + 2];
        float *a = A + ((size_t)n * J + j) * 12;
#pragma unroll
        for (int r = 0; r < 3; ++r) {
            a[r * 4 + 0] = g[r * 4 + 0];
            a[r * 4 + 1] = g[r * 4 + 1];
            a[r * 4 + 2] = g[r * 4 + 2];
            a[r * 4 + 3] = g[r * 4 + 3] - (g[r * 4] * jx + g[r * 4 + 1] * jy + g[r * 4 + 2] * jz);
            jtr[((size_t)n * J + j) * 3 + r] = g[r * 4 + 3] + trans[n * 3 + r];
        }
    }
}

constexpr int FT = 32, VT = 64, NTC = 3 * VT;
constexpr int BT = 256;
constexpr int FM = FT / 16;
constexpr int STS = NTC + 1;
constexpr int SF = 16;
constexpr int TBF = 10, TBV = 4;

template <int NG>
__global__ __launch_bounds__(BT) void smpl_blend_skin_kernel(const idf_smpl_model m, const float *__restrict__ feat,
                                                              const float *__restrict__ A, const float *__restrict__ trans,
                                                              int64_t N, float *__restrict__ verts,
                                                              float *__restrict__ v_posed) {
    extern __shared__ __attribute__((aligned(16))) float sm[];
    idf_args_now(m.V, m.J, m.S, m.blend, m.skin_idx, m.skin_w, feat, A, trans, N, verts, v_posed, gridDim.x);
    constexpr int KB = 16 * NG, nq = KB / 4;
    const int V = m.V, J = m.J, S = m.S;
    float *As = sm, *stage = sm;
    const int tid = threadIdx.x, lane = tid & 63, wave = (tid >> 6) & 3, fh = tid >> 8, li = lane & 15, kq = lane >> 4;
    const int nft = (int)((N + FT - 1) / FT), nvt = (V + VT - 1) / VT;
    const int nwg = gridDim.x, id = blockIdx.x;
    const int xq = nwg >> 3, xr = nwg & 7, xcd = id & 7;
    const int lid = (xcd < xr ? xcd * (xq + 1) : xr * (xq + 1) + (xcd - xr) * xq) + (id >> 3);
    const int blk = lid / (TBF * TBV), wi = lid - blk * (TBF * TBV);
    const int nvb = (nvt + TBV - 1) / TBV;
    const int ftile = blk / nvb * TBF + wi % TBF, vtile = blk % nvb * TBV + wi / TBF;
    if (ftile >= nft || vtile >= nvt) return;
    const int64_t f0 = (int64_t)ftile * FT;
    const int v0 = vtile * VT;
    IDF_SMPL_STAMP(0);

    {
        const uint32_t as_lds = idf_lds_addr(As);
        const int ncell = FT * nq;
        for (int i = wave; i * 64 < ncell; i += BT / 64) {
            const int p = min(i * 64 + lane, ncell - 1), row = p / nq, pos = p - row * nq;
            idf_dma16_v(feat + (size_t)min(f0 + row, N - 1) * KB + ((pos ^ ((row >> 1) & 7)) << 2), as_lds + (uint32_t)(i * 1024));
        }
    }
    const int vl = tid & 63, vme = v0 + vl;
    float sw[4];
    int so[4];
#pragma unroll
    for (int k = 0; k < 4; ++k) {
        const size_t e = (size_t)min(vme, V - 1) * S + min(k, S - 1);
        sw[k] = m.skin_w[e];
        so[k] = m.skin_idx[e] * 12;
    }
#pragma unroll
    for (int k = 0; k < 4; ++k) {
        const bool ok = k < S && vme < V;
        sw[k] = ok ? sw[k] : 0.f;
        so[k] = ok ? so[k] : 0;
    }
    asm volatile("s_waitcnt vmcnt(0)" ::: "memory");
    __syncthreads();
    IDF_SMPL_STAMP(1);

    const float *brow[3];
#pragma unroll
    for (int t = 0; t < 3; ++t) brow[t] = m.blend + ((size_t)((vtile * 4 + wave) * 3 + t) * NG * 64 + lane) * 4;
    f32x4 acc[FM][3];
#pragma unroll
    for (int i = 0; i < FM; ++i)
#pragma unroll
        for (int t = 0; t < 3; ++t) acc[i][t] = f32x4{0.f, 0.f, 0.f, 0.f};
    constexpr int PD = 3;
    float4 bq[PD + 1][3];
    auto ldg = [&](float4 (&dst)[3], int gi) {
#pragma unroll
        for (int t = 0; t < 3; ++t) dst[t] = *reinterpret_cast<const float4 *>(brow[t] + gi * 256);
    };
    auto mac = [&](const float4 (&bc)[3], int gi) {
#pragma unroll
        for (int i = 0; i < FM; ++i) {
            const int row = (fh * FM + i) * 16 + li;
            const float4 a = *reinterpret_cast<const float4 *>(As + row * KB + (((gi * 4 + kq) ^ ((row >> 1) & 7)) << 2));
#pragma unroll
            for (int t = 0; t < 3; ++t) acc[i][t] = __builtin_amdgcn_mfma_f32_16x16x4f32(a.x, bc[t].x, acc[i][t], 0, 0, 0);
#pragma unroll
            for (int t = 0; t < 3; ++t) acc[i][t] = __builtin_amdgcn_mfma_f32_16x16x4f32(a.y, bc[t].y, acc[i][t], 0, 0, 0);
#pragma unroll
            for (int t = 0; t < 3; ++t) acc[i][t] = __builtin_amdgcn_mfma_f32_16x16x4f32(a.z, bc[t].z, acc[i][t], 0, 0, 0);
#pragma unroll
            for (int t = 0; t < 3; ++t) acc[i][t] = __builtin_amdgcn_mfma_f32_16x16x4f32(a.w, bc[t].w, acc[i][t], 0, 0, 0);
        }
    };
#pragma unroll
    for (int g = 0; g < PD && g < NG; ++g) ldg(bq[g], g);
#pragma unroll
    for (int g = 0; g < NG; ++g) {
        if (g + PD < NG) ldg(bq[(g + PD) % (PD + 1)], g + PD);
        __builtin_amdgcn_sched_barrier(0);
        mac(bq[g % (PD + 1)], g);
        __builtin_amdgcn_sched_barrier(0);
    }
    __syncthreads();
    IDF_SMPL_STAMP(2);
#pragma unroll
    for (int i = 0; i < FM; ++i)
#pragma unroll
        for (int t = 0; t < 3; ++t)
#pragma unroll
            for (int r = 0; r < 4; ++r) stage[((fh * FM + i) * 16 + kq * 4 + r) * STS + (wave * 3 + t) * 16 + li] = acc[i][t][r];

    float *Asub = sm + ((FT * STS + 255) & ~255);
    float *ost = Asub + ((SF * J * 12 + 255) & ~255);
    float *trs = ost + SF * NTC;
    const int arow = J * 12;
    if (tid < FT * 3) trs[tid] = trans[min(f0 + tid / 3, N - 1) * 3 + tid % 3];
    for (int sub = 0; sub < FT / SF; ++sub) {
        const int64_t fs = f0 + sub * SF;
        if (fs >= N) break;
        __syncthreads();
        {
            const uint32_t asub_lds = idf_lds_addr(Asub);
            const float *src = idf_uniform_ptr(A + (size_t)fs * arow);
            for (int i = wave; i * 256 < SF * arow; i += BT / 64) idf_dma16_s(src + (size_t)i * 256, (uint32_t)(lane << 4), asub_lds + (uint32_t)(i * 1024));
            asm volatile("s_waitcnt vmcnt(0)" ::: "memory");
        }
        __syncthreads();
        IDF_SMPL_STAMP(3 + 3 * sub);
#pragma unroll
        for (int k = 0; k < SF * VT / BT; ++k) {
            const int f = (tid >> 6) + (BT / 64) * k, fr = sub * SF + f;
            const float px = stage[fr * STS + 3 * vl], py = stage[fr * STS + 3 * vl + 1], pz = stage[fr * STS + 3 * vl + 2];
            float4 t0 = make_float4(0.f, 0.f, 0.f, 0.f), t1 = t0, t2 = t0;
            const float *Af = Asub + f * arow;
#pragma unroll
            for (int b = 0; b < 4; ++b) {
                if (b < S) {
                    const float w = sw[b];
                    const float4 *a = reinterpret_cast<const float4 *>(Af + so[b]);
                    const float4 a0 = a[0], a1 = a[1], a2 = a[2];
                    t0.x = fmaf(w, a0.x, t0.x); t0.y = fmaf(w, a0.y, t0.y); t0.z = fmaf(w, a0.z, t0.z); t0.w = fmaf(w, a0.w, t0.w);
                    t1.x = fmaf(w, a1.x, t1.x); t1.y = fmaf(w, a1.y, t1.y); t1.z = fmaf(w, a1.z, t1.z); t1.w = fmaf(w, a1.w, t1.w);
                    t2.x = fmaf(w, a2.x, t2.x); t2.y = fmaf(w, a2.y, t2.y); t2.z = fmaf(w, a2.z, t2.z); t2.w = fmaf(w, a2.w, t2.w);
                }
            }
            float *o = ost + f * NTC + 3 * vl;
            o[0] = fmaf(t0.x, px, fmaf(t0.y, py, fmaf(t0.z, pz, t0.w))) + trs[fr * 3 + 0];
            o[1] = fmaf(t1.x, px, fmaf(t1.y, py, fmaf(t1.z, pz, t1.w))) + trs[fr * 3 + 1];
            o[2] = fmaf(t2.x, px, fmaf(t2.y, py, fmaf(t2.z, pz, t2.w))) + trs[fr * 3 + 2];
        }
        __syncthreads();
        IDF_SMPL_STAMP(4 + 3 * sub);
        const int nvalid = min(VT, V - v0) * 3;
        for (int idx = tid; idx < SF * (NTC / 2); idx += BT) {
            const int f = idx / (NTC / 2), c2 = (idx - f * (NTC / 2)) * 2;
            if (fs + f >= N || c2 >= nvalid) continue;
            const size_t go = ((size_t)(fs + f) * V + v0) * 3 + c2;
            *reinterpret_cast<float2 *>(verts + go) = *reinterpret_cast<const float2 *>(ost + f * NTC + c2);
            if (v_posed) *reinterpret_cast<float2 *>(v_posed + go) = make_float2(stage[(sub * SF + f) * STS + c2], stage[(sub * SF + f) * STS + c2 + 1]);
        }
        IDF_SMPL_STAMP(5 + 3 * sub);
    }
}

}

extern "C" size_t interdiff_smpl_workspace_bytes(const idf_smpl_model *m, int64_t N) {
    if (!m || N < 0) return 0;
    return idf_align((size_t)N * m->KB * sizeof(float)) + idf_align(((size_t)N + SF) * m->J * 12 * sizeof(float));
}

extern "C" int interdiff_smpl_forward(const idf_smpl_model *m, const float *pose, const float *betas, const float *trans,
                                      int64_t N, float *verts, float *jtr, float *v_posed, void *ws, size_t ws_bytes,
                                      void *stream) {
    if (!m || !pose || !betas || !trans || !verts || !jtr || !ws || N < 0) return IDF_E_INVAL;
    if (m->J < 1 || m->J > MAXJ || m->KB % 16 != 0 || m->KB < 9 * (m->J - 1) + m->n_betas + 1 || m->S < 1) return IDF_E_INVAL;
    if (ws_bytes < interdiff_smpl_workspace_bytes(m, N)) return IDF_E_NOMEM;
    if (N == 0) return IDF_OK;
    hipStream_t s = idf_stream(stream);
    float *feat = reinterpret_cast<float *>(ws);
    float *A = reinterpret_cast<float *>(reinterpret_cast<char *>(ws) + idf_align((size_t)N * m->KB * sizeof(float)));
    idf_prof_mark(IDF_K_SMPL_POSE, s);
    hipLaunchKernelGGL(smpl_pose_kernel, dim3((unsigned)N), dim3(64), 0, s, *m, pose, betas, trans, feat, A, jtr);
    const size_t lds = std::max((size_t)FT * m->KB, (size_t)((FT * STS + 255) & ~255) + ((SF * m->J * 12 + 255) & ~255) + (size_t)SF * NTC + FT * 3) * sizeof(float);
    if (lds > 150 * 1024 || m->KB % 32 != 0 || (m->V * 3) % 2 != 0 || m->S > 4) return IDF_E_INVAL;
    if (m->KB != 480) return IDF_E_INVAL;
    static std::atomic<uint64_t> lds_ok{0};
    if (lds > 64 * 1024 && idf_opt_in_lds(reinterpret_cast<const void *>(smpl_blend_skin_kernel<30>), 150 * 1024, lds_ok) != IDF_OK) return IDF_E_LAUNCH;
    idf_prof_mark(IDF_K_SMPL_BLEND_SKIN, s);
    const unsigned nwg_launch = (unsigned)(idf_cdiv(idf_cdiv(N, FT), TBF) * idf_cdiv(idf_cdiv(m->V, VT), TBV) * TBF * TBV);
    hipLaunchKernelGGL(smpl_blend_skin_kernel<30>, dim3(nwg_launch), dim3(BT), lds, s, *m,
                       feat, A, trans, N, verts, v_posed);
    idf_prof_mark(-1, s);
    IDF_CHECK_LAUNCH();
    return IDF_OK;
}
```

interdiff_amd/diffusion.py:

```python
import itertools
import math
import os
from types import SimpleNamespace
import numpy as np
import torch
from . import _lib


def get_named_beta_schedule(schedule_name, num_diffusion_timesteps, scale_betas=1.):
    n = num_diffusion_timesteps
    if schedule_name == 'linear':
        scale = scale_betas * 1000 / n
        return np.linspace(scale * 0.0001, scale * 0.02, n, dtype=np.float64)
    if schedule_name == 'cosine':
        abar = lambda t: math.cos((t + 0.008) / 1.008 * math.pi / 2) ** 2
        return np.array([min(1 - abar((i + 1) / n) / abar(i / n), 0.999) for i in range(n)], dtype=np.float64)
    raise NotImplementedError('unknown beta schedule: %s' % schedule_name)


GRAPH_BLOCKS = (49, 7, 1)
SPLIT_MAX_BATCH = int(os.environ.get('INTERDIFF_SPLIT_MAX_BATCH', 128))
N_CHAINS = int(os.environ.get('INTERDIFF_CHAINS', 2))
STAGGER_STEPS = int(os.environ.get('INTERDIFF_STAGGER', 0))
MAX_GRAPH_SHAPES = 8
_UID = itertools.count(1)


def fresh_seed():
    return int(torch.randint(0, 2 ** 62, (1,), dtype=torch.int64).item())


class GaussianDiffusion:

    def __init__(self, betas):
        betas = np.array(betas, dtype=np.float64)
        assert betas.ndim == 1 and (betas > 0).all() and (betas <= 1).all()
        self.betas = betas
        self.num_timesteps = int(betas.shape[0])
        alphas = 1.0 - betas
        self.alphas_cumprod = np.cumprod(alphas, axis=0)
        self.alphas_cumprod_prev = np.append(1.0, self.alphas_cumprod[:-1])
        self.posterior_variance = betas * (1.0 - self.alphas_cumprod_prev) / (1.0 - self.alphas_cumprod)
        self.posterior_log_variance_clipped = np.log(np.append(self.posterior_variance[1], self.posterior_variance[1:]))
        self.posterior_mean_coef1 = betas * np.sqrt(self.alphas_cumprod_prev) / (1.0 - self.alphas_cumprod)
        self.posterior_mean_coef2 = (1.0 - self.alphas_cumprod_prev) * np.sqrt(alphas) / (1.0 - self.alphas_cumprod)
        self._c1 = self.posterior_mean_coef1.astype(np.float32)
        self._c2 = self.posterior_mean_coef2.astype(np.float32)
        self._sigma = np.exp(np.float32(0.5) * self.posterior_log_variance_clipped.astype(np.float32)).astype(np.float32)
        self._t_cache = {}
        self._tables = {}
        self.fuse_plain_step = True
        self.chain_plain_steps = os.environ.get('INTERDIFF_CHAIN_STEPS', '1') != '0'
        self.split_chains = True
        self.split_min_rows = None
        self.stagger_steps = STAGGER_STEPS
        self._uid = next(_UID)

    def _timesteps(self, B, device):
        key = (B, str(device))
        if key not in self._t_cache:
            self._t_cache[key] = torch.arange(self.num_timesteps, device=device, dtype=torch.int64)[:, None].repeat(1, B).contiguous()
        return self._t_cache[key]

    def _table(self, device):
        key = str(device)
        if key not in self._tables:
            sig = self._sigma.copy()
            sig[0] = 0.0
            blend = (np.arange(self.num_timesteps, dtype=np.float32) / np.float32(1000)).astype(np.float32)
            self._tables[key] = torch.from_numpy(np.stack([self._c1, self._c2, sig, blend], axis=1).astype(np.float32)).contiguous().to(device)
        return self._tables[key]

    def _graph_loop(self, model, img, model_kwargs, denoised_fn, seed, todo, dump_steps, t_start, shard=None):
        lib = _lib.load()
        y = model_kwargs.get('y', {})
        B, dev = img.shape[0], img.device
        first, total = (0, B) if shard is None else shard
        per_clip = img.numel() // B
        elem0 = first * per_clip
        rows = total * img.shape[-1]
        table = self._table(dev)
        has_mask = 'inpainting_mask' in y and 'inpainted_motion' in y
        mu8 = gc = None
        if has_mask:
            m = y['inpainting_mask']
            assert img.shape == m.shape == y['inpainted_motion'].shape
            mu8, gc = (m if m.dtype == torch.uint8 else m.view(torch.uint8)).contiguous(), y['inpainted_motion'].contiguous()
        cond = y['cond']
        cache = model.__dict__.setdefault('_graph_cache', {})
        key = (self._uid, tuple(img.shape), has_mask, tuple(cond.shape), model.ffn_graph_key(rows) if hasattr(model, 'ffn_graph_key') else 0)
        st = cache.get(key)
        if st is None:
            st = SimpleNamespace(x=torch.zeros_like(img), x0=torch.empty_like(img), ts=torch.zeros(B, dtype=torch.int64, device=dev),
                                 state=torch.zeros(8, dtype=torch.int64, device=dev), cond=torch.empty_like(cond, memory_format=torch.contiguous_format),
                                 gt=torch.empty_like(img) if has_mask else None,
                                 mask=torch.empty(img.shape, dtype=torch.uint8, device=dev) if has_mask else None, graphs={})
            st.kwargs = {'y': {'cond': st.cond}}
            if len(cache) >= MAX_GRAPH_SHAPES:
                evicted = list(cache.values())
                cache.clear()
                if hasattr(model, 'forget_shape_buffers'):
                    for old in evicted:
                        model.forget_shape_buffers(getattr(old, 'pool_keys', ()))
            cache[key] = st
            fresh = True
            pools_before = None
        else:
            fresh = False
        st.cond.copy_(cond)
        if has_mask:
            st.gt.copy_(gc)
            st.mask.copy_(mu8)
        if fresh and hasattr(model, 'shape_buffer_keys'):
            pools_before = model.shape_buffer_keys()
        model.prepare_memory(st.cond)
        rows_kw = {'batch_rows': rows} if getattr(model, 'accepts_batch_rows', False) else {}
        if fresh:
            model(st.x, st.ts, out=st.x0, **st.kwargs, **rows_kw)
            if getattr(model, 'supports_forward_step', False):
                scratch = SimpleNamespace(x=st.x.clone(), ts=st.ts.clone(), state=torch.tensor([2, 0, 1, 0, 0, 0, 0, 0], dtype=torch.int64, device=dev))
                model.forward_step(scratch.x, scratch.ts, table, scratch.state, gt=st.gt, mask=st.mask, **st.kwargs, **rows_kw)
                if getattr(model, 'step_chaining', False):
                    scratch.state.copy_(torch.tensor([2, 0, 1, 0, 0, 0, 0, 0], dtype=torch.int64))
                    scratch.ts.copy_(st.ts)
                    model.forward_step(scratch.x, scratch.ts, table, scratch.state, gt=st.gt, mask=st.mask, embed_next=True, **st.kwargs, **rows_kw)
                    model.forward_step(scratch.x, scratch.ts, table, scratch.state, gt=st.gt, mask=st.mask, embed_ready=True, **st.kwargs, **rows_kw)
            torch.cuda.synchronize(dev)
            if pools_before is not None:
                st.pool_keys = model.shape_buffer_keys() - pools_before

        def posterior(x, x0, g, mk, st):
            _lib.check(lib.interdiff_posterior_step_dev(_lib.dptr(x), _lib.dptr(x0), _lib.dptr(g, allow_none=True),
                                                        _lib.dptr(mk, allow_none=True), x.numel(), _lib.dptr(table), _lib.dptr(st.state),
                                                        _lib.dptr(st.ts), B, _lib.stream()), 'posterior_step_dev')

        fused = self.fuse_plain_step and getattr(model, 'supports_forward_step', False)
        nch = N_CHAINS
        split = (fused and self.split_chains and nch > 1 and 2 * nch <= B <= SPLIT_MAX_BATCH
                 and B * img.shape[-1] > ((model.one_chain_max_rows() if hasattr(model, 'one_chain_max_rows') else getattr(model, 'FFN16_MAX_ROWS', 0)) if self.split_min_rows is None else self.split_min_rows))
        if split and not hasattr(st, 'chains'):
            st.chains = []
            for c in range(nch):
                start = c * (B // nch) + min(c, B % nch)
                h = B // nch + (1 if c < B % nch else 0)
                sl = slice(start, start + h)
                st.chains.append(SimpleNamespace(
                    sl=sl, x=st.x[sl], ts=st.ts[sl], gt=st.gt[sl] if has_mask else None, mask=st.mask[sl] if has_mask else None,
                    state=st.state if c == 0 else torch.zeros(8, dtype=torch.int64, device=dev),
                    cond=torch.empty(cond.shape[0], h, cond.shape[2], device=dev),
                    memctx=torch.empty(model.memctx_floats(h, cond.shape[0]) if getattr(model, 'accepts_batch_rows', False) else model.memctx_floats(h), dtype=torch.float32, device=dev),
                    ws=torch.empty(model.workspace_bytes(h, img.shape[-1]), dtype=torch.uint8, device=dev), stream=torch.cuda.Stream(dev)))
        if split:
            for ch in st.chains:
                ch.cond.copy_(st.cond[:, ch.sl])
                model.prepare_memory(ch.cond, into=ch.memctx)

        chain_steps = self.chain_plain_steps and fused and getattr(model, 'step_chaining', False)
        if st.__dict__.get('chain_steps') != chain_steps:
            st.graphs.clear()
            st.chain_steps = chain_steps

        def enqueue_plain(k):
            link = lambda i: dict(embed_ready=i > 0, embed_next=i + 1 < k) if chain_steps else {}
            if split:
                cur = torch.cuda.current_stream()
                for ch in st.chains:
                    ch.stream.wait_stream(cur)
                    with torch.cuda.stream(ch.stream):
                        for i in range(k):
                            model.forward_step(ch.x, ch.ts, table, ch.state, gt=ch.gt, mask=ch.mask, memctx=ch.memctx, ws=ch.ws, batch_rows=rows, **link(i))
                for ch in st.chains:
                    cur.wait_stream(ch.stream)
            else:
                for i in range(k):
                    if fused:
                        model.forward_step(st.x, st.ts, table, st.state, gt=st.gt, mask=st.mask, **link(i), **st.kwargs, **rows_kw)
                    else:
                        model(st.x, st.ts, out=st.x0, **st.kwargs, **rows_kw)
                        posterior(st.x, st.x0, st.gt, st.mask, st)

        def graph_of(k):
            if (k, fused, split) not in st.graphs:
                g = torch.cuda.CUDAGraph()
                with torch.cuda.graph(g):
                    enqueue_plain(k)
                st.graphs[(k, fused, split)] = g
            return st.graphs[(k, fused, split)]

        staggered = split and self.stagger_steps > 0 and B % nch == 0 and denoised_fn is not None and hasattr(denoised_fn, 'slice_kwargs')
        hook_dev = (not staggered and denoised_fn is not None and getattr(denoised_fn, 'graph_capturable', False) and getattr(denoised_fn, 'debug', None) is None
                    and getattr(denoised_fn, 'is_active', None) is not None and all(k in y for k in ('inpainted_motion', 'hand_pose', 'beta', 'obj_points'))
                    and os.environ.get('INTERDIFF_EAGER_HOOK') != '1')
        if hook_dev:
            hooks = st.__dict__.setdefault('hooks', {})
            hk = hooks.get(denoised_fn._uid)
            shapes = tuple(tuple(y[k].shape) for k in ('hand_pose', 'beta', 'obj_points'))
            if hk is None or hk.shapes != shapes:
                hk = SimpleNamespace(shapes=shapes, ws=denoised_fn.workspace_for(B, img.shape[-1]), fresh=True,
                                     y=dict(inpainted_motion=st.gt if has_mask else torch.empty_like(img),
                                            **{k: torch.empty(y[k].shape, dtype=torch.float32, device=dev) for k in ('hand_pose', 'beta', 'obj_points')}))
                hooks[denoised_fn._uid] = hk
                for stale in [gk for gk in st.graphs if isinstance(gk, tuple) and gk[0] == 'hook' and gk[1] == denoised_fn._uid]:
                    del st.graphs[stale]
            for k in ('hand_pose', 'beta', 'obj_points') + (() if has_mask else ('inpainted_motion',)):
                hk.y[k].copy_(y[k])
            if hk.fresh:
                denoised_fn.apply_dev(hk.y['inpainted_motion'].clone(), table, torch.zeros(8, dtype=torch.int64, device=dev), hk.y, hk.ws)
                torch.cuda.synchronize(dev)
                hk.fresh = False

        def hook_graph(k):
            key = ('hook', denoised_fn._uid, k, fused, split)
            if key not in st.graphs:
                g = torch.cuda.CUDAGraph()
                with torch.cuda.graph(g):
                    if k:
                        enqueue_plain(k)
                    model(st.x, st.ts, out=st.x0, **st.kwargs, **rows_kw)
                    if has_mask:
                        _lib.check(lib.interdiff_inpaint(_lib.dptr(st.x0), _lib.dptr(st.gt), _lib.dptr(st.mask), st.x0.numel(), _lib.stream()), 'inpaint')
                    denoised_fn.apply_dev(st.x0, table, st.state, hk.y, hk.ws)
                    posterior(st.x, st.x0, None, None, st)
                    if split:
                        for ch in st.chains[1:]:
                            ch.state[:6].copy_(st.state[:6])
                st.graphs[key] = g
            return st.graphs[key]
        st.x.copy_(img)
        if elem0 % 4:
            raise ValueError('a shard must start at a multiple of 4 elements (C * T = %d per clip)' % per_clip)
        st.state.copy_(torch.tensor([t_start, 0, int(seed) & 0x7FFFFFFFFFFFFFFF, 0, 0, 0, elem0, 0], dtype=torch.int64))
        gate = getattr(denoised_fn, 'is_active', None)
        active = lambda i: denoised_fn is not None and (gate is None or gate(i))
        if staggered:
            return self._staggered_chains(model, st, table, model_kwargs, denoised_fn, active, seed, todo, dump_steps, t_start, has_mask, rows, elem0)
        if split:
            for c, ch in enumerate(st.chains[1:], 1):
                ch.state.copy_(torch.tensor([t_start, 0, int(seed) & 0x7FFFFFFFFFFFFFFF, 0, 0, 0, elem0 + ch.sl.start * per_clip, 0], dtype=torch.int64))
        st.ts.fill_(t_start)
        ts_all = self._timesteps(B, dev)
        dump, it, i, end = [], 0, t_start, t_start - todo
        while i > end:
            if active(i) and hook_dev:
                hook_graph(0).replay()
                k = 1
            elif active(i):
                if 'fwd' not in st.graphs:
                    g = torch.cuda.CUDAGraph()
                    with torch.cuda.graph(g):
                        model(st.x, st.ts, out=st.x0, **st.kwargs, **rows_kw)
                    st.graphs['fwd'] = g
                st.graphs['fwd'].replay()
                x0 = st.x0
                if has_mask:
                    _lib.check(lib.interdiff_inpaint(_lib.dptr(x0), _lib.dptr(st.gt), _lib.dptr(st.mask), x0.numel(), _lib.stream()), 'inpaint')
                t = ts_all[i]
                t.host_value = i
                x0 = denoised_fn(x0, t, model_kwargs).contiguous()
                posterior(st.x, x0, None, None, st)
                if split:
                    for ch in st.chains[1:]:
                        ch.state[:6].copy_(st.state[:6])
                k = 1
            else:
                run = 1
                while i - run > end and not active(i - run) and not (dump_steps is not None and (it + run - 1) in dump_steps):
                    run += 1
                k = next(b for b in GRAPH_BLOCKS if b <= run)
                if (hook_dev and k == run and i - run > end and active(i - run)
                        and not (dump_steps is not None and (it + k - 1) in dump_steps)):
                    hook_graph(k).replay()
                    k += 1
                else:
                    graph_of(k).replay()
            i -= k
            it += k
            if dump_steps is not None and (it - 1) in dump_steps:
                dump.append(st.x.clone())
        return dump if dump_steps is not None else st.x.clone()

    def _staggered_chains(self, model, st, table, model_kwargs, denoised_fn, active, seed, todo, dump_steps, t_start, has_mask, rows, elem0):
        lib = _lib.load()
        dev, B = st.x.device, st.x.shape[0]
        chains, h = st.chains, st.x.shape[0] // len(st.chains)
        end = t_start - todo
        prog, i, it = [], t_start, 0
        lag_at = self.stagger_steps if todo > self.stagger_steps else 0
        while i > end:
            if active(i):
                prog.append(('hook', i))
                k = 1
            else:
                run = 1
                while (i - run > end and not active(i - run) and not (dump_steps is not None and (it + run - 1) in dump_steps)
                       and it + run != lag_at):
                    run += 1
                k = next(b for b in GRAPH_BLOCKS if b <= run)
                prog.append(('plain', k))
            i -= k
            it += k
            if it == lag_at:
                prog.append(('lag',))
            if dump_steps is not None and (it - 1) in dump_steps:
                prog.append(('dump',))
        n_lag = next((j + 1 for j, op in enumerate(prog) if op[0] == 'lag'), 1 if prog else 0)
        cur = torch.cuda.current_stream(dev)
        need_k = sorted({op[1] for op in prog if op[0] == 'plain'})
        need_fwd = any(op[0] == 'hook' for op in prog)
        for c, ch in enumerate(chains):
            if not hasattr(ch, 'x0'):
                ch.x0, ch.graphs = st.x0[ch.sl], {}
            for k in need_k:
                if k not in ch.graphs:
                    g = torch.cuda.CUDAGraph()
                    with torch.cuda.graph(g):
                        for _ in range(k):
                            model.forward_step(ch.x, ch.ts, table, ch.state, gt=ch.gt, mask=ch.mask, memctx=ch.memctx, ws=ch.ws, batch_rows=rows)
                    ch.graphs[k] = g
            if need_fwd and 'fwd' not in ch.graphs:
                g = torch.cuda.CUDAGraph()
                with torch.cuda.graph(g):
                    model(ch.x, ch.ts, out=ch.x0, memctx=ch.memctx, ws=ch.ws, batch_rows=rows)
                ch.graphs['fwd'] = g
        for c, ch in enumerate(chains):
            ch.state.copy_(torch.tensor([t_start, 0, int(seed) & 0x7FFFFFFFFFFFFFFF, 0, 0, 0, elem0 + c * ch.x.numel(), 0], dtype=torch.int64))
        st.ts.fill_(t_start)
        ts_all = self._timesteps(B, dev)
        kw = [denoised_fn.slice_kwargs(model_kwargs, ch.sl) for ch in chains] if need_fwd else None
        dumps = [torch.empty_like(st.x) for op in prog if op[0] == 'dump']

        def run_op(c, ch, op, n_dump):
            if op[0] == 'plain':
                ch.graphs[op[1]].replay()
            elif op[0] == 'hook':
                i = op[1]
                ch.graphs['fwd'].replay()
                if has_mask:
                    _lib.check(lib.interdiff_inpaint(_lib.dptr(ch.x0), _lib.dptr(ch.gt), _lib.dptr(ch.mask), ch.x0.numel(), _lib.stream()), 'inpaint')
                t = ts_all[i][ch.sl]
                t.host_value = i
                x0 = denoised_fn(ch.x0, t, kw[c]).contiguous()
                _lib.check(lib.interdiff_posterior_step_dev(_lib.dptr(ch.x), _lib.dptr(x0), None, None, ch.x.numel(), _lib.dptr(table),
                                                            _lib.dptr(ch.state), _lib.dptr(ch.ts), h, _lib.stream()), 'posterior_step_dev')
            elif op[0] == 'dump':
                dumps[n_dump][ch.sl].copy_(ch.x)
            elif op[0] == 'lag' and c + 1 < len(chains):
                ch.lag_event = torch.cuda.Event()
                ch.lag_event.record()

        n_dump = [0] * len(chains)
        for ch in chains:
            ch.stream.wait_stream(cur)
        for j in range(len(prog) + n_lag * (len(chains) - 1)):
            for c, ch in enumerate(chains):
                jj = j - c * n_lag
                if not 0 <= jj < len(prog):
                    continue
                with torch.cuda.stream(ch.stream):
                    if jj == 0 and c > 0 and getattr(chains[c - 1], 'lag_event', None) is not None:
                        ch.stream.wait_event(chains[c - 1].lag_event)
                    run_op(c, ch, prog[jj], n_dump[c])
                    if prog[jj][0] == 'dump':
                        n_dump[c] += 1
        for ch in chains:
            cur.wait_stream(ch.stream)
            ch.lag_event = None
        return dumps if dump_steps is not None else st.x.clone()

    def _step(self, model, img, x0_buf, i, it, t, model_kwargs, denoised_fn, noise_i, seed, elem0=0, rows_kw={}):
        lib = _lib.load()
        y = model_kwargs.get('y', {})
        x0 = model(img, t, **model_kwargs, **rows_kw)
        if 'inpainting_mask' in y and 'inpainted_motion' in y:
            m, g = y['inpainting_mask'], y['inpainted_motion']
            assert x0.shape == m.shape == g.shape
            mu8, gc = (m if m.dtype == torch.uint8 else m.view(torch.uint8)).contiguous(), g.contiguous()
            _lib.check(lib.interdiff_inpaint(_lib.dptr(x0, torch.float32), _lib.dptr(gc, torch.float32), _lib.dptr(mu8),
                                             x0.numel(), _lib.stream()), 'inpaint')
        if denoised_fn is not None:
            x0 = denoised_fn(x0, t, model_kwargs)
        sigma = 0.0 if i == 0 else float(self._sigma[i])
        _lib.check(lib.interdiff_posterior_step_at(_lib.dptr(img, torch.float32), _lib.dptr(x0, torch.float32),
                                                   _lib.dptr(noise_i, torch.float32, allow_none=True), img.numel(),
                                                   float(self._c1[i]), float(self._c2[i]), sigma, seed, it, elem0, _lib.stream()),
                   'posterior_step')
        return x0

    def p_sample_loop(self, model, shape, noise=None, clip_denoised=True, denoised_fn=None, cond_fn=None, model_kwargs=None,
                      device=None, progress=False, skip_timesteps=0, init_image=None, randomize_class=False,
                      cond_fn_with_grad=False, dump_steps=None, const_noise=False, step_noise=None, seed=None, n_steps=None,
                      use_graph=True, first_t=None, shard=None):
        if clip_denoised:
            raise NotImplementedError('clip_denoised=True is not used on the eval path (eval_smpl_short.py:153)')
        if cond_fn is not None or skip_timesteps or init_image is not None or randomize_class or cond_fn_with_grad or const_noise:
            raise NotImplementedError('only noise=, denoised_fn=, model_kwargs=, dump_steps= are live (SURVEY.md §8(b))')
        if model_kwargs is None:
            model_kwargs = {}
        if seed is None:
            seed = fresh_seed()
        if device is None:
            device = next(model.parameters()).device
        assert isinstance(shape, (tuple, list))
        if shard is not None:
            shard = (int(shard[0]), int(shard[1]))
            if not 0 <= shard[0] <= shard[0] + shape[0] <= shard[1]:
                raise ValueError('shard=(first_clip, total_clips) must contain this batch of %d clips' % shape[0])
        first, total = (0, shape[0]) if shard is None else shard
        per_clip = int(np.prod(shape[1:]))
        elem0 = first * per_clip
        if shard is not None and elem0 % 4:
            raise ValueError('a shard must start at a multiple of 4 elements (C * T = %d per clip)' % per_clip)
        if noise is not None:
            img = noise.clone().contiguous().float()
        else:
            lib = _lib.load()
            img = torch.empty(*shape, dtype=torch.float32, device=device)
            _lib.check(lib.interdiff_randn_at(_lib.dptr(img), img.numel(), seed, 0xFFFFFFFF, elem0, _lib.stream()), 'randn')
            y = model_kwargs.get('y', {})
            if 'inpainting_mask' in y and 'inpainted_motion' in y:
                m = y['inpainting_mask']
                mu8, gc = (m if m.dtype == torch.uint8 else m.view(torch.uint8)).contiguous(), y['inpainted_motion'].contiguous()
                _lib.check(lib.interdiff_inpaint(_lib.dptr(img), _lib.dptr(gc), _lib.dptr(mu8), img.numel(), _lib.stream()), 'inpaint')
        t_first = self.num_timesteps - 1 if first_t is None else int(first_t)
        if not 0 <= t_first < self.num_timesteps:
            raise ValueError('first_t outside the schedule')
        todo = t_first + 1 if n_steps is None else min(int(n_steps), t_first + 1)
        if (step_noise is None and use_graph and getattr(model, 'graph_safe', False) and img.is_cuda
                and 'cond' in model_kwargs.get('y', {}) and os.environ.get('INTERDIFF_NO_GRAPH') != '1'):
            return self._graph_loop(model, img, model_kwargs, denoised_fn, seed, todo, dump_steps, t_first, shard)
        rows_kw = {'batch_rows': total * shape[-1]} if shard is not None and getattr(model, 'accepts_batch_rows', False) else {}
        ts = self._timesteps(shape[0], device)
        dump = []
        cond = model_kwargs.get('y', {}).get('cond') if isinstance(model_kwargs.get('y', None), dict) else None
        if cond is not None and hasattr(model, 'prepare_memory'):
            model.prepare_memory(cond)
        for it, i in enumerate(range(t_first, t_first - todo, -1)):
            t = ts[i]
            t.host_value = i
            if step_noise is None:
                nz = None
            elif callable(step_noise):
                nz = step_noise(it, img).contiguous()
            else:
                nz = step_noise[it]
            self._step(model, img, None, i, it, t, model_kwargs, denoised_fn, nz, seed, elem0, rows_kw)
            if dump_steps is not None and it in dump_steps:
                dump.append(img.clone())
        return dump if dump_steps is not None else img


class SpacedDiffusion(GaussianDiffusion):

    def __init__(self, use_timesteps, betas):
        base = GaussianDiffusion(betas)
        use = set(use_timesteps)
        last, new_betas, self.timestep_map = 1.0, [], []
        for i, ac in enumerate(base.alphas_cumprod):
            if i in use:
                new_betas.append(1 - ac / last)
                last = ac
                self.timestep_map.append(i)
        if self.timestep_map != list(range(len(betas))):
            raise NotImplementedError('timestep respacing is not used by the reference eval path')
        super().__init__(np.array(new_betas))


def create_gaussian_diffusion(noise_schedule='cosine', diffusion_steps=1000):
    betas = get_named_beta_schedule(noise_schedule, diffusion_steps, 1.)
    return SpacedDiffusion(range(diffusion_steps), betas)
```

interdiff_amd/smpl.py:

```python
import ctypes as C
import numpy as np
import torch
from . import _lib


def _np(a):
    return a.detach().cpu().numpy() if isinstance(a, torch.Tensor) else np.asarray(a)


def pack_smpl_model(model, device):
    vt = _np(model['v_template']).astype(np.float64).reshape(-1, 3)
    sdirs = _np(model['shapedirs']).astype(np.float64)
    pdirs = _np(model['posedirs']).astype(np.float64)
    jreg = _np(model['J_regressor']).astype(np.float64)
    wts = _np(model['weights']).astype(np.float32)
    parents = _np(model['parents']).astype(np.int64).copy()
    V, J, nb = vt.shape[0], wts.shape[1], sdirs.shape[2]
    kp = 9 * (J - 1)
    if pdirs.shape != (V, 3, kp) or jreg.shape != (J, V):
        raise ValueError('inconsistent SMPL buffers')
    KB = (kp + nb + 1 + 15) // 16 * 16
    blend = np.zeros((3 * V, KB), np.float32)
    blend[:, :kp] = pdirs.reshape(3 * V, kp)
    blend[:, kp:kp + nb] = sdirs.reshape(3 * V, nb)
    blend[:, kp + nb] = vt.reshape(3 * V)
    jt = (jreg @ vt).astype(np.float32)
    js = np.einsum('jv,vck->jck', jreg, sdirs).astype(np.float32)
    nnz = (wts != 0)
    S = max(1, int(nnz.sum(1).max()))
    skin_idx = np.zeros((V, S), np.int32)
    skin_w = np.zeros((V, S), np.float32)
    for v in range(V):
        js_ = np.nonzero(nnz[v])[0]
        skin_idx[v, :len(js_)] = js_
        skin_w[v, :len(js_)] = wts[v, js_]
    parents[0] = 0
    t = lambda a: torch.from_numpy(np.ascontiguousarray(a)).to(device)
    nvt = -(-V // 64)
    rows = np.zeros((nvt * 192, KB), np.float32)
    rows[:3 * V] = blend
    frag = rows.reshape(nvt, 4, 3, 16, KB // 16, 4, 4).transpose(0, 1, 2, 4, 5, 3, 6)
    bufs = dict(blend=t(frag), blend_rows=t(blend), jt=t(jt), js=t(js), parents=t(parents.astype(np.int32)), skin_idx=t(skin_idx), skin_w=t(skin_w))
    m = _lib.SmplModel()
    m.V, m.J, m.n_betas, m.KB, m.S = V, J, nb, KB, S
    for k, v in bufs.items():
        if k != 'blend_rows':
            setattr(m, k, v.data_ptr())
    return m, bufs


class SMPL_Layer:
    def __init__(self, model, device='cuda'):
        self.lib = _lib.load()
        self.device = torch.device(device)
        self.cmodel, self._bufs = pack_smpl_model(model, self.device)
        self.th_faces = torch.from_numpy(_np(model['faces']).astype(np.int64)).to(self.device)
        self.v_template = _np(model['v_template']).astype(np.float32).reshape(-1, 3)
        self.num_joints = self.cmodel.J
        self.kintree_parents = [int(p) for p in _np(model['parents'])]
        self._ws = None

    def _workspace(self, N):
        need = self.lib.interdiff_smpl_workspace_bytes(C.byref(self.cmodel), N)
        if self._ws is None or self._ws.numel() < need:
            self._ws = torch.empty(max(need, 256), dtype=torch.uint8, device=self.device)
        return self._ws

    def forward(self, th_pose_axisang, th_betas=None, th_trans=None, th_offsets=None, scale=1., want_v_posed=True):
        if th_offsets is not None or scale != 1.:
            raise NotImplementedError('th_offsets / scale are not used on the eval_smpl_short path')
        N = th_pose_axisang.shape[0]
        J, V, nb = self.cmodel.J, self.cmodel.V, self.cmodel.n_betas
        if th_pose_axisang.shape[1] != 3 * J:
            raise ValueError('pose must be [N,%d]' % (3 * J))
        if th_betas is None:
            th_betas = torch.zeros(N, nb, device=self.device)
        if th_trans is None:
            th_trans = torch.zeros(N, 3, device=self.device)
        pose, betas, trans = (a.contiguous().float() for a in (th_pose_axisang, th_betas, th_trans))
        verts = torch.empty(N, V, 3, dtype=torch.float32, device=self.device)
        jtr = torch.empty(N, J, 3, dtype=torch.float32, device=self.device)
        v_posed = torch.empty(N, V, 3, dtype=torch.float32, device=self.device) if want_v_posed else None
        ws = self._workspace(N)
        _lib.check(self.lib.interdiff_smpl_forward(C.byref(self.cmodel), _lib.dptr(pose, torch.float32), _lib.dptr(betas, torch.float32),
                                                   _lib.dptr(trans, torch.float32), N, _lib.dptr(verts), _lib.dptr(jtr),
                                                   _lib.dptr(v_posed, allow_none=True), _lib.dptr(ws), ws.numel(), _lib.stream()),
                   'smpl_forward')
        return verts, jtr, v_posed, v_posed

    __call__ = forward
```

Baseline: 7.185 million.

## Precompute per-sample SMPL hand/shape blend base and point order outside denoising steps

Reorders the SMPL blend-shape columns so the body-joint pose features come first in a fixed block of 192. Hand joints, betas and template form a constant tail that depends only on per-sample inputs. A new begin_sample entry point computes the blend base for that constant tail and the object point ordering once per sample. Each denoising step then runs a smaller blend-skin kernel over only the per-step columns and adds the stored base, skipping the point-order kernel. This adds workspace state that must stay valid across the steps of a sample, plus an extra pose-kernel pass and new templated kernel variants.

```diff
diff --git a/include/interdiff_hip.h b/include/interdiff_hip.h
--- a/include/interdiff_hip.h
+++ b/include/interdiff_hip.h
@@ -37,6 +37,11 @@
 int interdiff_smpl_forward(const idf_smpl_model *m, const float *pose, const float *betas,
                            const float *trans, int64_t N, float *verts, float *jtr,
                            float *v_posed, void *ws, size_t ws_bytes, void *stream);
+int interdiff_smpl_base(const idf_smpl_model *m, const float *pose, const float *betas, int64_t N,
+                        void *ws, size_t ws_bytes, void *stream);
+int interdiff_smpl_forward_prepared(const idf_smpl_model *m, const float *pose, const float *betas,
+                                    const float *trans, int64_t N, float *verts, float *jtr,
+                                    float *v_posed, void *ws, size_t ws_bytes, void *stream);
 
 int interdiff_vertex_normals(const float *verts, int64_t N, int32_t V, const int32_t *faces,
                              const int32_t *adj_ptr, const int32_t *adj_face,
@@ -189,6 +194,12 @@
 int interdiff_correction_dev(const idf_correction_ctx *c, float *x0, const float *gt, const float *hand_pose,
                              const float *beta, const float *obj_points, int32_t B, int32_t T, const float *table,
                              const int64_t *state, void *ws, size_t ws_bytes, void *stream);
+
+int interdiff_correction_begin_sample(const idf_correction_ctx *c, const float *gt, const float *hand_pose, const float *beta,
+                                      const float *obj_points, int32_t B, int32_t T, void *ws, size_t ws_bytes, void *stream);
+int interdiff_correction_step(const idf_correction_ctx *c, float *x0, const float *gt, const float *hand_pose, const float *beta,
+                              const float *obj_points, int32_t B, int32_t T, float blend_t, const float *table, const int64_t *state,
+                              uint8_t *condition, int32_t *contact, float *distance, float *loss, void *ws, size_t ws_bytes, void *stream);
 
 #define IDF_CONTACT_STATS 12
 size_t interdiff_contact_nn_workspace_bytes(const idf_correction_ctx *c, int32_t B, int32_t T);
diff --git a/interdiff_amd/_lib.py b/interdiff_amd/_lib.py
--- a/interdiff_amd/_lib.py
+++ b/interdiff_amd/_lib.py
@@ -88,6 +88,8 @@
     'interdiff_rotation_6d_to_axis_angle': (C.c_int, [vp, vp, i64, vp]),
     'interdiff_smpl_workspace_bytes': (sz, [C.POINTER(SmplModel), i64]),
     'interdiff_smpl_forward': (C.c_int, [C.POINTER(SmplModel), vp, vp, vp, i64, vp, vp, vp, vp, sz, vp]),
+    'interdiff_smpl_base': (C.c_int, [C.POINTER(SmplModel), vp, vp, i64, vp, sz, vp]),
+    'interdiff_smpl_forward_prepared': (C.c_int, [C.POINTER(SmplModel), vp, vp, vp, i64, vp, vp, vp, vp, sz, vp]),
     'interdiff_vertex_normals': (C.c_int, [vp, i64, i32, vp, vp, vp, vp, vp, vp]),
     'interdiff_nn_argmin': (C.c_int, [vp, i32, vp, i32, i64, vp, vp]),
     'interdiff_point2point_signed': (C.c_int, [vp, i32, vp, i32, i64, vp, vp, vp, vp, vp, vp, vp, vp, vp]),
@@ -116,6 +118,9 @@
     'interdiff_correction': (C.c_int, [C.POINTER(CorrectionCtx), vp, vp, vp, vp, vp, i32, i32, f32,
                                        vp, vp, vp, vp, vp, sz, vp]),
     'interdiff_correction_dev': (C.c_int, [C.POINTER(CorrectionCtx), vp, vp, vp, vp, vp, i32, i32, vp, vp, vp, sz, vp]),
+    'interdiff_correction_begin_sample': (C.c_int, [C.POINTER(CorrectionCtx), vp, vp, vp, vp, i32, i32, vp, sz, vp]),
+    'interdiff_correction_step': (C.c_int, [C.POINTER(CorrectionCtx), vp, vp, vp, vp, vp, i32, i32, f32, vp, vp,
+                                            vp, vp, vp, vp, vp, sz, vp]),
     'interdiff_metrics_workspace_bytes': (sz, [C.POINTER(CorrectionCtx), i32, i32]),
     'interdiff_metrics': (C.c_int, [C.POINTER(CorrectionCtx), vp, vp, vp, vp, vp, vp, vp, vp, i32, i32, i32,
                                     vp, vp, sz, vp]),
diff --git a/interdiff_amd/correction.py b/interdiff_amd/correction.py
--- a/interdiff_amd/correction.py
+++ b/interdiff_amd/correction.py
@@ -52,14 +52,26 @@
     def workspace_for(self, B, T):
         return torch.empty(self.lib.interdiff_correction_workspace_bytes(C.byref(self.ctx), B, T), dtype=torch.uint8, device=self.device)
 
-    def apply_dev(self, x, table, state, y, ws):
+    def begin_sample(self, y, ws):
+        B, _, Cc, T = y['inpainted_motion'].shape
+        if y['obj_points'].shape[1] != self.ctx.n_points:
+            raise ValueError('obj_points must have %d points' % self.ctx.n_points)
+        _lib.check(self.lib.interdiff_correction_begin_sample(C.byref(self.ctx), _lib.dptr(y['inpainted_motion'], torch.float32),
+                                                              _lib.dptr(y['hand_pose'], torch.float32), _lib.dptr(y['beta'], torch.float32),
+                                                              _lib.dptr(y['obj_points'], torch.float32), B, T, _lib.dptr(ws), ws.numel(), _lib.stream()),
+                   'correction_begin_sample')
+
+    def apply_dev(self, x, table, state, y, ws, prepared=False):
         B, _, Cc, T = x.shape
         if y['obj_points'].shape[1] != self.ctx.n_points:
             raise ValueError('obj_points must have %d points' % self.ctx.n_points)
-        _lib.check(self.lib.interdiff_correction_dev(C.byref(self.ctx), _lib.dptr(x, torch.float32), _lib.dptr(y['inpainted_motion'], torch.float32),
-                                                     _lib.dptr(y['hand_pose'], torch.float32), _lib.dptr(y['beta'], torch.float32),
-                                                     _lib.dptr(y['obj_points'], torch.float32), B, T, _lib.dptr(table), _lib.dptr(state),
-                                                     _lib.dptr(ws), ws.numel(), _lib.stream()), 'correction_dev')
+        args = (C.byref(self.ctx), _lib.dptr(x, torch.float32), _lib.dptr(y['inpainted_motion'], torch.float32),
+                _lib.dptr(y['hand_pose'], torch.float32), _lib.dptr(y['beta'], torch.float32), _lib.dptr(y['obj_points'], torch.float32), B, T)
+        if prepared:
+            _lib.check(self.lib.interdiff_correction_step(*args, 0.0, _lib.dptr(table), _lib.dptr(state), None, None, None, None,
+                                                          _lib.dptr(ws), ws.numel(), _lib.stream()), 'correction_step')
+        else:
+            _lib.check(self.lib.interdiff_correction_dev(*args, _lib.dptr(table), _lib.dptr(state), _lib.dptr(ws), ws.numel(), _lib.stream()), 'correction_dev')
         return x
 
     def _workspace(self, B, T):
diff --git a/interdiff_amd/csrc/correction.hip b/interdiff_amd/csrc/correction.hip
--- a/interdiff_amd/csrc/correction.hip
+++ b/interdiff_amd/csrc/correction.hip
@@ -561,14 +561,15 @@
 
 int launch_contact(hipStream_t s, int64_t N, const float *verts, int V, const float *obj_points, int P, int32_t *porder,
                    const float *objR, const float *objT, const idf_correction_ctx *c, int B, float *markers, float *loss_sum,
-                   float *min_dist, int32_t *label, float *o2h, int32_t *idx, unsigned long long *stats, int64_t nn_from, const PredArgs *pred = nullptr) {
+                   float *min_dist, int32_t *label, float *o2h, int32_t *idx, unsigned long long *stats, int64_t nn_from, const PredArgs *pred = nullptr,
+                   bool order_ready = false ) {
     const int M = c->n_markers;
     const size_t lds = contact_lds_bytes(V);
     if (lds > 160 * 1024 - 16384 || P > MAXP) return IDF_E_INVAL;
     const bool ordered = c->vorder != nullptr;
     if (ordered != (c->faces_scan != nullptr) || ordered != (c->markers_scan != nullptr) || ordered != (c->adj_pair_scan != nullptr)) return IDF_E_INVAL;
     const int32_t *faces = ordered ? c->faces_scan : c->faces, *mpos = ordered ? c->markers_scan : c->markers_idx;
-    if (porder) hipLaunchKernelGGL(corr_point_order_kernel, dim3((unsigned)B), dim3(1024), 0, s, obj_points, P, porder);
+    if (porder && !order_ready) hipLaunchKernelGGL(corr_point_order_kernel, dim3((unsigned)B), dim3(1024), 0, s, obj_points, P, porder);
     if (pred) {
         const size_t lds2 = (pred->nclips > 0 && lds < idf_objproj_dev::OBJPROJ_LDS) ? idf_objproj_dev::OBJPROJ_LDS : lds;
         static std::atomic<uint64_t> lds_ok2{0};
@@ -772,24 +773,55 @@
     return carve(c, B, T, nullptr).total;
 }
 
+static int correction_check(const idf_correction_ctx *c, const float *gt, const float *hand_pose, const float *beta, const float *obj_points,
+                            int32_t B, int32_t T, const void *ws) {
+    if (!c || !c->smpl || !c->objproj || !gt || !hand_pose || !beta || !obj_points || !ws || B <= 0 || T <= 0) return IDF_E_INVAL;
+    const int M = c->n_markers, P = c->n_points;
+    if (c->smpl->J != 52 || c->smpl->n_betas != 10 || M > MAXM || M != c->objproj->P || P > MAXP || T != c->objproj->T ||
+        c->past_len != c->objproj->past_len || c->past_len >= T)
+        return IDF_E_INVAL;
+    return IDF_OK;
+}
+
+static int begin_sample_impl(const idf_correction_ctx *c, const float *gt, const float *hand_pose, const float *beta, const float *obj_points,
+                             int32_t B, int32_t T, void *ws, size_t ws_bytes, void *stream) {
+    if (const int rc = correction_check(c, gt, hand_pose, beta, obj_points, B, T, ws)) return rc;
+    CorrWs w = carve(c, B, T, ws);
+    if (ws_bytes < w.total) return IDF_E_NOMEM;
+    hipStream_t s = idf_stream(stream);
+    const int64_t N = (int64_t)B * T;
+    idf_prof_mark(IDF_K_CORR_PREPARE, s);
+    hipLaunchKernelGGL(corr_prepare_kernel, dim3((unsigned)idf_cdiv(N * 24, 256)), dim3(256), 0, s, gt, gt, hand_pose, B, T, w.pose,
+                       w.trans, w.objR, w.objT, w.gt_angles, w.gt_trans);
+    int rc = interdiff_smpl_base(c->smpl, w.pose, beta, N, w.smpl_ws, w.smpl_ws_bytes, stream);
+    if (rc) return rc;
+    idf_prof_mark(IDF_K_CORR_CONTACT, s);
+    rc = idf_point_order(s, obj_points, B, c->n_points, w.porder);
+    if (rc) return rc;
+    idf_prof_mark(-1, s);
+    IDF_CHECK_LAUNCH();
+    return IDF_OK;
+}
+
 static int correction_impl(const idf_correction_ctx *c, float *x0, const float *gt, const float *hand_pose,
                            const float *beta, const float *obj_points, int32_t B, int32_t T, float blend_t, const float *blend_table,
                            const int64_t *blend_state, uint8_t *condition, int32_t *contact, float *distance, float *loss, void *ws,
-                           size_t ws_bytes, void *stream) {
-    if (!c || !c->smpl || !c->objproj || !x0 || !gt || !hand_pose || !beta || !obj_points || !ws || B <= 0 || T <= 0) return IDF_E_INVAL;
+                           size_t ws_bytes, void *stream, bool prepared) {
+    if (!x0) return IDF_E_INVAL;
+    if (const int rc0 = correction_check(c, gt, hand_pose, beta, obj_points, B, T, ws)) return rc0;
     const int V = c->smpl->V, M = c->n_markers, P = c->n_points;
-    if (c->smpl->J != 52 || c->smpl->n_betas != 10 || M > MAXM || M != c->objproj->P || P > MAXP || T != c->objproj->T ||
-        c->past_len != c->objproj->past_len || c->past_len >= T)
-        return IDF_E_INVAL;
     CorrWs w = carve(c, B, T, ws);
     if (ws_bytes < w.total) return IDF_E_NOMEM;
+    if (!prepared) {
+        if (const int rc0 = begin_sample_impl(c, gt, hand_pose, beta, obj_points, B, T, ws, ws_bytes, stream)) return rc0;
+    }
     hipStream_t s = idf_stream(stream);
     const int64_t N = (int64_t)B * T;
     const bool fused = (c->tune & 2) == 0 && idf_objproj_check(c->objproj) == IDF_OK;
     idf_prof_mark(IDF_K_CORR_PREPARE, s);
     hipLaunchKernelGGL(corr_prepare_kernel, dim3((unsigned)idf_cdiv(N * 24, 256)), dim3(256), 0, s, x0, gt, hand_pose, B, T, w.pose,
                        w.trans, w.objR, w.objT, w.gt_angles, w.gt_trans);
-    int rc = interdiff_smpl_forward(c->smpl, w.pose, beta, w.trans, N, w.verts, w.jtr, nullptr, w.smpl_ws, w.smpl_ws_bytes, stream);
+    int rc = interdiff_smpl_forward_prepared(c->smpl, w.pose, beta, w.trans, N, w.verts, w.jtr, nullptr, w.smpl_ws, w.smpl_ws_bytes, stream);
     if (rc) return rc;
     idf_prof_mark(IDF_K_CORR_CONTACT, s);
     PredArgs pred{};
@@ -800,7 +832,7 @@
         pred.nclips = B;
     }
     rc = launch_contact(s, N, w.verts, V, obj_points, P, w.porder, w.objR, w.objT, c, B, fused ? nullptr : w.markers, w.loss_sum, w.min_dist, w.label, nullptr,
-                        nullptr, nullptr, (int64_t)c->past_len * B, &pred);
+                        nullptr, nullptr, (int64_t)c->past_len * B, &pred, true);
     if (rc) return rc;
     uint8_t *cond = condition ? condition : w.condition;
     int32_t *cont = contact ? contact : w.contact;
@@ -826,14 +858,26 @@
                                     const float *beta, const float *obj_points, int32_t B, int32_t T, float blend_t,
                                     uint8_t *condition, int32_t *contact, float *distance, float *loss, void *ws,
                                     size_t ws_bytes, void *stream) {
-    return correction_impl(c, x0, gt, hand_pose, beta, obj_points, B, T, blend_t, nullptr, nullptr, condition, contact, distance, loss, ws, ws_bytes, stream);
+    return correction_impl(c, x0, gt, hand_pose, beta, obj_points, B, T, blend_t, nullptr, nullptr, condition, contact, distance, loss, ws, ws_bytes, stream, false);
 }
 
 extern "C" int interdiff_correction_dev(const idf_correction_ctx *c, float *x0, const float *gt, const float *hand_pose,
                                         const float *beta, const float *obj_points, int32_t B, int32_t T, const float *table,
                                         const int64_t *state, void *ws, size_t ws_bytes, void *stream) {
     if (!table || !state) return IDF_E_INVAL;
-    return correction_impl(c, x0, gt, hand_pose, beta, obj_points, B, T, 0.f, table, state, nullptr, nullptr, nullptr, nullptr, ws, ws_bytes, stream);
+    return correction_impl(c, x0, gt, hand_pose, beta, obj_points, B, T, 0.f, table, state, nullptr, nullptr, nullptr, nullptr, ws, ws_bytes, stream, false);
+}
+
+extern "C" int interdiff_correction_begin_sample(const idf_correction_ctx *c, const float *gt, const float *hand_pose, const float *beta,
+                                                 const float *obj_points, int32_t B, int32_t T, void *ws, size_t ws_bytes, void *stream) {
+    return begin_sample_impl(c, gt, hand_pose, beta, obj_points, B, T, ws, ws_bytes, stream);
+}
+
+extern "C" int interdiff_correction_step(const idf_correction_ctx *c, float *x0, const float *gt, const float *hand_pose, const float *beta,
+                                         const float *obj_points, int32_t B, int32_t T, float blend_t, const float *table, const int64_t *state,
+                                         uint8_t *condition, int32_t *contact, float *distance, float *loss, void *ws, size_t ws_bytes, void *stream) {
+    if ((table == nullptr) != (state == nullptr)) return IDF_E_INVAL;
+    return correction_impl(c, x0, gt, hand_pose, beta, obj_points, B, T, blend_t, table, state, condition, contact, distance, loss, ws, ws_bytes, stream, true);
 }
 
 namespace {
diff --git a/interdiff_amd/csrc/smpl.hip b/interdiff_amd/csrc/smpl.hip
--- a/interdiff_amd/csrc/smpl.hip
+++ b/interdiff_amd/csrc/smpl.hip
@@ -9,11 +9,13 @@
 namespace {
 
 constexpr int MAXJ = 64;
+constexpr int JC = 22;
+constexpr int KC = 192;
 
 __global__ __launch_bounds__(64) void smpl_pose_kernel(const idf_smpl_model m, const float *__restrict__ pose,
                                                        const float *__restrict__ betas, const float *__restrict__ trans,
                                                        float *__restrict__ feat, float *__restrict__ A,
-                                                       float *__restrict__ jtr) {
+                                                       float *__restrict__ jtr, int part) {
     __shared__ float Rs[MAXJ * 9], Js[MAXJ * 3], Gs[MAXJ * 12];
     const int64_t n = blockIdx.x;
     const int j = threadIdx.x, J = m.J, nb = m.n_betas, KB = m.KB;
@@ -29,12 +31,17 @@
         }
     }
     float *f = feat + n * KB;
-    if (j >= 1 && j < J) {
-#pragma unroll
-        for (int e = 0; e < 9; ++e) f[(j - 1) * 9 + e] = Rs[j * 9 + e] - ((e == 0 || e == 4 || e == 8) ? 1.0f : 0.0f);
-    }
-    const int base = 9 * (J - 1);
-    for (int k = j; k < KB - base; k += 64) f[base + k] = k < nb ? beta[k] : (k == nb ? 1.0f : 0.0f);
+    if (j >= 1 && j < J && (j >= JC) == (part != 0)) {
+        float *fj = f + (j < JC ? (j - 1) * 9 : KC + (j - JC) * 9);
+#pragma unroll
+        for (int e = 0; e < 9; ++e) fj[e] = Rs[j * 9 + e] - ((e == 0 || e == 4 || e == 8) ? 1.0f : 0.0f);
+    }
+    if (part != 0) {
+        const int base = KC + 9 * (J - JC);
+        for (int k = j; k < KB - base; k += 64) f[base + k] = k < nb ? beta[k] : (k == nb ? 1.0f : 0.0f);
+        return;
+    }
+    for (int k = 9 * (JC - 1) + j; k < KC; k += 64) f[k] = 0.0f;
     __syncthreads();
     if (j < 12) {
         const int r = j >> 2, c = j & 3;
@@ -78,14 +85,14 @@
 constexpr int SF = 16;
 constexpr int TBF = 10, TBV = 4;
 
-template <int NG>
+template <int NG, int G0, int NGF, bool BASE, bool ADD = !BASE>
 __global__ __launch_bounds__(BT) void smpl_blend_skin_kernel(const idf_smpl_model m, const float *__restrict__ feat,
                                                               const float *__restrict__ A, const float *__restrict__ trans,
                                                               int64_t N, float *__restrict__ verts,
-                                                              float *__restrict__ v_posed) {
+                                                              float *__restrict__ v_posed, float *__restrict__ base) {
     extern __shared__ __attribute__((aligned(16))) float sm[];
-    idf_args_now(m.V, m.J, m.S, m.blend, m.skin_idx, m.skin_w, feat, A, trans, N, verts, v_posed, gridDim.x);
-    constexpr int KB = 16 * NG, nq = KB / 4;
+    idf_args_now(m.V, m.J, m.S, m.blend, m.skin_idx, m.skin_w, feat, A, trans, N, verts, v_posed, base, gridDim.x);
+    constexpr int KB = 16 * NG, nq = KB / 4, KBF = 16 * NGF;
     const int V = m.V, J = m.J, S = m.S;
     float *As = sm, *stage = sm;
     const int tid = threadIdx.x, lane = tid & 63, wave = (tid >> 6) & 3, fh = tid >> 8, li = lane & 15, kq = lane >> 4;
@@ -106,12 +113,23 @@
         const int ncell = FT * nq;
         for (int i = wave; i * 64 < ncell; i += BT / 64) {
             const int p = min(i * 64 + lane, ncell - 1), row = p / nq, pos = p - row * nq;
-            idf_dma16_v(feat + (size_t)min(f0 + row, N - 1) * KB + ((pos ^ ((row >> 1) & 7)) << 2), as_lds + (uint32_t)(i * 1024));
-        }
-    }
+            idf_dma16_v(feat + (size_t)min(f0 + row, N - 1) * KBF + G0 * 16 + ((pos ^ ((row >> 1) & 7)) << 2), as_lds + (uint32_t)(i * 1024));
+        }
+    }
+    float4 *btile = reinterpret_cast<float4 *>(base) + ((size_t)ftile * nvt + vtile) * (FM * 3 * BT) + tid;
+    f32x4 acc[FM][3];
+    float4 b4[FM][3];
+#pragma unroll
+    for (int i = 0; i < FM; ++i)
+#pragma unroll
+        for (int t = 0; t < 3; ++t) {
+            acc[i][t] = f32x4{0.f, 0.f, 0.f, 0.f};
+            if constexpr (ADD) b4[i][t] = btile[(i * 3 + t) * BT];
+        }
     const int vl = tid & 63, vme = v0 + vl;
-    float sw[4];
-    int so[4];
+    float sw[4] = {0.f, 0.f, 0.f, 0.f};
+    int so[4] = {0, 0, 0, 0};
+    if constexpr (!BASE)
 #pragma unroll
     for (int k = 0; k < 4; ++k) {
         const size_t e = (size_t)min(vme, V - 1) * S + min(k, S - 1);
@@ -130,12 +148,7 @@
 
     const float *brow[3];
 #pragma unroll
-    for (int t = 0; t < 3; ++t) brow[t] = m.blend + ((size_t)((vtile * 4 + wave) * 3 + t) * NG * 64 + lane) * 4;
-    f32x4 acc[FM][3];
-#pragma unroll
-    for (int i = 0; i < FM; ++i)
-#pragma unroll
-        for (int t = 0; t < 3; ++t) acc[i][t] = f32x4{0.f, 0.f, 0.f, 0.f};
+    for (int t = 0; t < 3; ++t) brow[t] = m.blend + (((size_t)((vtile * 4 + wave) * 3 + t) * NGF + G0) * 64 + lane) * 4;
     constexpr int PD = 3;
     float4 bq[PD + 1][3];
     auto ldg = [&](float4 (&dst)[3], int gi) {
@@ -166,6 +179,20 @@
         mac(bq[g % (PD + 1)], g);
         __builtin_amdgcn_sched_barrier(0);
     }
+    if constexpr (BASE) {
+#pragma unroll
+        for (int i = 0; i < FM; ++i)
+#pragma unroll
+            for (int t = 0; t < 3; ++t) btile[(i * 3 + t) * BT] = make_float4(acc[i][t][0], acc[i][t][1], acc[i][t][2], acc[i][t][3]);
+        return;
+    }
+    if constexpr (ADD)
+#pragma unroll
+    for (int i = 0; i < FM; ++i)
+#pragma unroll
+        for (int t = 0; t < 3; ++t) {
+            acc[i][t][0] += b4[i][t].x; acc[i][t][1] += b4[i][t].y; acc[i][t][2] += b4[i][t].z; acc[i][t][3] += b4[i][t].w;
+        }
     __syncthreads();
     IDF_SMPL_STAMP(2);
 #pragma unroll
@@ -230,32 +257,95 @@
 
 }
 
+namespace {
+
+size_t smpl_base_bytes(const idf_smpl_model *m, int64_t N) {
+    return (size_t)idf_cdiv(N, FT) * idf_cdiv(m->V, VT) * FT * NTC * sizeof(float);
+}
+
+struct SmplWs { float *feat, *A, *base; };
+SmplWs smpl_carve(const idf_smpl_model *m, int64_t N, void *ws) {
+    char *p = reinterpret_cast<char *>(ws);
+    const size_t o1 = idf_align((size_t)N * m->KB * sizeof(float)), o2 = o1 + idf_align(((size_t)N + SF) * m->J * 12 * sizeof(float));
+    return SmplWs{reinterpret_cast<float *>(p), reinterpret_cast<float *>(p + o1), reinterpret_cast<float *>(p + o2)};
+}
+
+int smpl_check(const idf_smpl_model *m, int64_t N, const void *ws, size_t ws_bytes) {
+    if (!m || !ws || N < 0) return IDF_E_INVAL;
+    if (m->J <= JC || m->J > MAXJ || m->KB % 16 != 0 || m->KB < KC + 9 * (m->J - JC) + m->n_betas + 1 || m->S < 1) return IDF_E_INVAL;
+    if (m->KB != 480) return IDF_E_INVAL;
+    if ((m->V * 3) % 2 != 0 || m->S > 4) return IDF_E_INVAL;
+    if (ws_bytes < interdiff_smpl_workspace_bytes(m, N)) return IDF_E_NOMEM;
+    return IDF_OK;
+}
+
+constexpr int NGF = 30, NGC = KC / 16, NGB = NGF - NGC;
+
+unsigned smpl_grid(const idf_smpl_model *m, int64_t N) { return (unsigned)(idf_cdiv(idf_cdiv(N, FT), TBF) * idf_cdiv(idf_cdiv(m->V, VT), TBV) * TBF * TBV); }
+
+}
+
 extern "C" size_t interdiff_smpl_workspace_bytes(const idf_smpl_model *m, int64_t N) {
     if (!m || N < 0) return 0;
-    return idf_align((size_t)N * m->KB * sizeof(float)) + idf_align(((size_t)N + SF) * m->J * 12 * sizeof(float));
+    return idf_align((size_t)N * m->KB * sizeof(float)) + idf_align(((size_t)N + SF) * m->J * 12 * sizeof(float)) + idf_align(smpl_base_bytes(m, N));
+}
+
+extern "C" int interdiff_smpl_base(const idf_smpl_model *m, const float *pose, const float *betas, int64_t N, void *ws, size_t ws_bytes, void *stream) {
+    if (!pose || !betas) return IDF_E_INVAL;
+    if (const int rc = smpl_check(m, N, ws, ws_bytes)) return rc;
+    if (N == 0) return IDF_OK;
+    hipStream_t s = idf_stream(stream);
+    const SmplWs w = smpl_carve(m, N, ws);
+    idf_prof_mark(IDF_K_SMPL_POSE, s);
+    hipLaunchKernelGGL(smpl_pose_kernel, dim3((unsigned)N), dim3(64), 0, s, *m, pose, betas, nullptr, w.feat, nullptr, nullptr, 1);
+    idf_prof_mark(IDF_K_SMPL_BLEND_SKIN, s);
+    hipLaunchKernelGGL((smpl_blend_skin_kernel<NGB, NGC, NGF, true>), dim3(smpl_grid(m, N)), dim3(BT), (size_t)FT * NGB * 16 * sizeof(float), s, *m,
+                       w.feat, nullptr, nullptr, N, nullptr, nullptr, w.base);
+    idf_prof_mark(-1, s);
+    IDF_CHECK_LAUNCH();
+    return IDF_OK;
+}
+
+extern "C" int interdiff_smpl_forward_prepared(const idf_smpl_model *m, const float *pose, const float *betas, const float *trans,
+                                               int64_t N, float *verts, float *jtr, float *v_posed, void *ws, size_t ws_bytes,
+                                               void *stream) {
+    if (!pose || !betas || !trans || !verts || !jtr) return IDF_E_INVAL;
+    if (const int rc = smpl_check(m, N, ws, ws_bytes)) return rc;
+    if (N == 0) return IDF_OK;
+    hipStream_t s = idf_stream(stream);
+    const SmplWs w = smpl_carve(m, N, ws);
+    idf_prof_mark(IDF_K_SMPL_POSE, s);
+    hipLaunchKernelGGL(smpl_pose_kernel, dim3((unsigned)N), dim3(64), 0, s, *m, pose, betas, trans, w.feat, w.A, jtr, 0);
+    const size_t lds = std::max((size_t)FT * KC, (size_t)((FT * STS + 255) & ~255) + ((SF * m->J * 12 + 255) & ~255) + (size_t)SF * NTC + FT * 3) * sizeof(float);
+    if (lds > 150 * 1024) return IDF_E_INVAL;
+    static std::atomic<uint64_t> lds_ok{0};
+    if (lds > 64 * 1024 && idf_opt_in_lds(reinterpret_cast<const void *>(smpl_blend_skin_kernel<NGC, 0, NGF, false>), 150 * 1024, lds_ok) != IDF_OK) return IDF_E_LAUNCH;
+    idf_prof_mark(IDF_K_SMPL_BLEND_SKIN, s);
+    hipLaunchKernelGGL((smpl_blend_skin_kernel<NGC, 0, NGF, false>), dim3(smpl_grid(m, N)), dim3(BT), lds, s, *m,
+                       w.feat, w.A, trans, N, verts, v_posed, w.base);
+    idf_prof_mark(-1, s);
+    IDF_CHECK_LAUNCH();
+    return IDF_OK;
 }
 
 extern "C" int interdiff_smpl_forward(const idf_smpl_model *m, const float *pose, const float *betas, const float *trans,
                                       int64_t N, float *verts, float *jtr, float *v_posed, void *ws, size_t ws_bytes,
                                       void *stream) {
-    if (!m || !pose || !betas || !trans || !verts || !jtr || !ws || N < 0) return IDF_E_INVAL;
-    if (m->J < 1 || m->J > MAXJ || m->KB % 16 != 0 || m->KB < 9 * (m->J - 1) + m->n_betas + 1 || m->S < 1) return IDF_E_INVAL;
-    if (ws_bytes < interdiff_smpl_workspace_bytes(m, N)) return IDF_E_NOMEM;
+    if (!pose || !betas || !trans || !verts || !jtr) return IDF_E_INVAL;
+    if (const int rc = smpl_check(m, N, ws, ws_bytes)) return rc;
     if (N == 0) return IDF_OK;
     hipStream_t s = idf_stream(stream);
-    float *feat = reinterpret_cast<float *>(ws);
-    float *A = reinterpret_cast<float *>(reinterpret_cast<char *>(ws) + idf_align((size_t)N * m->KB * sizeof(float)));
+    const SmplWs w = smpl_carve(m, N, ws);
     idf_prof_mark(IDF_K_SMPL_POSE, s);
-    hipLaunchKernelGGL(smpl_pose_kernel, dim3((unsigned)N), dim3(64), 0, s, *m, pose, betas, trans, feat, A, jtr);
+    hipLaunchKernelGGL(smpl_pose_kernel, dim3((unsigned)N), dim3(64), 0, s, *m, pose, betas, nullptr, w.feat, nullptr, nullptr, 1);
+    hipLaunchKernelGGL(smpl_pose_kernel, dim3((unsigned)N), dim3(64), 0, s, *m, pose, betas, trans, w.feat, w.A, jtr, 0);
     const size_t lds = std::max((size_t)FT * m->KB, (size_t)((FT * STS + 255) & ~255) + ((SF * m->J * 12 + 255) & ~255) + (size_t)SF * NTC + FT * 3) * sizeof(float);
-    if (lds > 150 * 1024 || m->KB % 32 != 0 || (m->V * 3) % 2 != 0 || m->S > 4) return IDF_E_INVAL;
-    if (m->KB != 480) return IDF_E_INVAL;
+    if (lds > 150 * 1024) return IDF_E_INVAL;
     static std::atomic<uint64_t> lds_ok{0};
-    if (lds > 64 * 1024 && idf_opt_in_lds(reinterpret_cast<const void *>(smpl_blend_skin_kernel<30>), 150 * 1024, lds_ok) != IDF_OK) return IDF_E_LAUNCH;
+    if (lds > 64 * 1024 && idf_opt_in_lds(reinterpret_cast<const void *>(smpl_blend_skin_kernel<NGF, 0, NGF, false, false>), 150 * 1024, lds_ok) != IDF_OK) return IDF_E_LAUNCH;
     idf_prof_mark(IDF_K_SMPL_BLEND_SKIN, s);
-    const unsigned nwg_launch = (unsigned)(idf_cdiv(idf_cdiv(N, FT), TBF) * idf_cdiv(idf_cdiv(m->V, VT), TBV) * TBF * TBV);
-    hipLaunchKernelGGL(smpl_blend_skin_kernel<30>, dim3(nwg_launch), dim3(BT), lds, s, *m,
-                       feat, A, trans, N, verts, v_posed);
+    hipLaunchKernelGGL((smpl_blend_skin_kernel<NGF, 0, NGF, false, false>), dim3(smpl_grid(m, N)), dim3(BT), lds, s, *m,
+                       w.feat, w.A, trans, N, verts, v_posed, w.base);
     idf_prof_mark(-1, s);
     IDF_CHECK_LAUNCH();
     return IDF_OK;
diff --git a/interdiff_amd/diffusion.py b/interdiff_amd/diffusion.py
--- a/interdiff_amd/diffusion.py
+++ b/interdiff_amd/diffusion.py
@@ -204,8 +204,12 @@
                     del st.graphs[stale]
             for k in ('hand_pose', 'beta', 'obj_points') + (() if has_mask else ('inpainted_motion',)):
                 hk.y[k].copy_(y[k])
+            prepared = hasattr(denoised_fn, 'begin_sample')
+            if prepared:
+                denoised_fn.begin_sample(hk.y, hk.ws)
+            hook_kw = dict(prepared=True) if prepared else {}
             if hk.fresh:
-                denoised_fn.apply_dev(hk.y['inpainted_motion'].clone(), table, torch.zeros(8, dtype=torch.int64, device=dev), hk.y, hk.ws)
+                denoised_fn.apply_dev(hk.y['inpainted_motion'].clone(), table, torch.zeros(8, dtype=torch.int64, device=dev), hk.y, hk.ws, **hook_kw)
                 torch.cuda.synchronize(dev)
                 hk.fresh = False
 
@@ -219,7 +223,7 @@
                     model(st.x, st.ts, out=st.x0, **st.kwargs, **rows_kw)
                     if has_mask:
                         _lib.check(lib.interdiff_inpaint(_lib.dptr(st.x0), _lib.dptr(st.gt), _lib.dptr(st.mask), st.x0.numel(), _lib.stream()), 'inpaint')
-                    denoised_fn.apply_dev(st.x0, table, st.state, hk.y, hk.ws)
+                    denoised_fn.apply_dev(st.x0, table, st.state, hk.y, hk.ws, **hook_kw)
                     posterior(st.x, st.x0, None, None, st)
                     if split:
                         for ch in st.chains[1:]:
diff --git a/interdiff_amd/smpl.py b/interdiff_amd/smpl.py
--- a/interdiff_amd/smpl.py
+++ b/interdiff_amd/smpl.py
@@ -6,6 +6,19 @@
 
 def _np(a):
     return a.detach().cpu().numpy() if isinstance(a, torch.Tensor) else np.asarray(a)
+
+
+JC, KC = 22, 192
+
+
+def blend_columns(J, nb):
+    kp, nc = 9 * (J - 1), 9 * (min(J, JC) - 1)
+    if nc > KC:
+        raise ValueError('per-call columns do not fit')
+    src_call = np.arange(nc)
+    src_const = np.arange(nc, kp + nb + 1)
+    KBK = KC + (len(src_const) + 15) // 16 * 16
+    return (src_call, src_call.copy()), (src_const, KC + np.arange(len(src_const))), KBK
 
 
 def pack_smpl_model(model, device):
@@ -36,13 +49,15 @@
         skin_w[v, :len(js_)] = wts[v, js_]
     parents[0] = 0
     t = lambda a: torch.from_numpy(np.ascontiguousarray(a)).to(device)
+    (cs, cd), (ks, kd), KBK = blend_columns(J, nb)
     nvt = -(-V // 64)
-    rows = np.zeros((nvt * 192, KB), np.float32)
-    rows[:3 * V] = blend
-    frag = rows.reshape(nvt, 4, 3, 16, KB // 16, 4, 4).transpose(0, 1, 2, 4, 5, 3, 6)
+    rows = np.zeros((nvt * 192, KBK), np.float32)
+    rows[:3 * V, cd] = blend[:, cs]
+    rows[:3 * V, kd] = blend[:, ks]
+    frag = rows.reshape(nvt, 4, 3, 16, KBK // 16, 4, 4).transpose(0, 1, 2, 4, 5, 3, 6)
     bufs = dict(blend=t(frag), blend_rows=t(blend), jt=t(jt), js=t(js), parents=t(parents.astype(np.int32)), skin_idx=t(skin_idx), skin_w=t(skin_w))
     m = _lib.SmplModel()
-    m.V, m.J, m.n_betas, m.KB, m.S = V, J, nb, KB, S
+    m.V, m.J, m.n_betas, m.KB, m.S = V, J, nb, KBK, S
     for k, v in bufs.items():
         if k != 'blend_rows':
             setattr(m, k, v.data_ptr())
@@ -66,7 +81,16 @@
             self._ws = torch.empty(max(need, 256), dtype=torch.uint8, device=self.device)
         return self._ws
 
-    def forward(self, th_pose_axisang, th_betas=None, th_trans=None, th_offsets=None, scale=1., want_v_posed=True):
+    def prepare(self, th_pose_axisang, th_betas=None):
+        N = th_pose_axisang.shape[0]
+        if th_betas is None:
+            th_betas = torch.zeros(N, self.cmodel.n_betas, device=self.device)
+        pose, betas = th_pose_axisang.contiguous().float(), th_betas.contiguous().float()
+        ws = self._workspace(N)
+        _lib.check(self.lib.interdiff_smpl_base(C.byref(self.cmodel), _lib.dptr(pose, torch.float32), _lib.dptr(betas, torch.float32), N,
+                                                _lib.dptr(ws), ws.numel(), _lib.stream()), 'smpl_base')
+
+    def forward(self, th_pose_axisang, th_betas=None, th_trans=None, th_offsets=None, scale=1., want_v_posed=True, prepared=False):
         if th_offsets is not None or scale != 1.:
             raise NotImplementedError('th_offsets / scale are not used on the eval_smpl_short path')
         N = th_pose_axisang.shape[0]
@@ -82,9 +106,10 @@
         jtr = torch.empty(N, J, 3, dtype=torch.float32, device=self.device)
         v_posed = torch.empty(N, V, 3, dtype=torch.float32, device=self.device) if want_v_posed else None
         ws = self._workspace(N)
-        _lib.check(self.lib.interdiff_smpl_forward(C.byref(self.cmodel), _lib.dptr(pose, torch.float32), _lib.dptr(betas, torch.float32),
-                                                   _lib.dptr(trans, torch.float32), N, _lib.dptr(verts), _lib.dptr(jtr),
-                                                   _lib.dptr(v_posed, allow_none=True), _lib.dptr(ws), ws.numel(), _lib.stream()),
+        fn = self.lib.interdiff_smpl_forward_prepared if prepared else self.lib.interdiff_smpl_forward
+        _lib.check(fn(C.byref(self.cmodel), _lib.dptr(pose, torch.float32), _lib.dptr(betas, torch.float32),
+                      _lib.dptr(trans, torch.float32), N, _lib.dptr(verts), _lib.dptr(jtr),
+                      _lib.dptr(v_posed, allow_none=True), _lib.dptr(ws), ws.numel(), _lib.stream()),
                    'smpl_forward')
         return verts, jtr, v_posed, v_posed
 
```

New measurement: 6.873 million. 4.4% lower.
